# NetLogo-Mobile/Phy-Engine

Hardware: AMD Instinct MI355X
Metric: transient steps/sec (+ Newton iters/sec), 10k-node RC mesh (higher is better)
Workload: dtype f64

## Files before the change

### include/pe_hip.h

```cpp
#ifndef PE_HIP_H
#define PE_HIP_H

#include <stddef.h>
#include <stdint.h>

#ifdef __cplusplus
extern "C" {
#endif

typedef struct pe_hip_engine pe_hip_engine;

enum pe_hip_status
{
    PE_HIP_OK = 0,
    PE_HIP_ERR_ARG = -1,
    PE_HIP_ERR_NO_DEVICE = -2,
    PE_HIP_ERR_SINGULAR = -3,
    PE_HIP_ERR_NO_CONVERGENCE = -4,
    PE_HIP_ERR_INTERNAL = -5,
    PE_HIP_ERR_INACCURATE = -6
};

enum pe_hip_kind
{
// ... 59 lines not shown
} pe_hip_timings;

typedef struct pe_hip_info
{
    int rows, n_nodes, n_branches, batch;
    int nnz_a;
    long long nnz_lu;
    long long nnz_lu_stored;
    int n_fronts, max_front, tree_depth, n_row_swaps;
    double factor_flops;
    long long bytes_per_instance;
    int n_r, n_c, n_l, n_v, n_i, n_d;
    int nonlinear;
    int n_parts;
    int n_top_levels;
    int n_wavefronts;
    int lds_bytes;
    long long nnz_lu_stored_top;
    int n_wave_fronts;
    int n_quad_fronts;
    long long nnz_lu_stored_quad;
    int mid_top_limit, ew_grid, quad_lds_pad;
} pe_hip_info;

typedef struct pe_hip_run_stats
{
    long long steps;
    long long newton_iters;
    double gpu_ms;
    int n_launches;
    int n_failed;
    double dominant_ms;
    int dominant_launches;
} pe_hip_run_stats;

int pe_hip_device_count(void);
int pe_hip_create(int device, pe_hip_engine** out);
void pe_hip_destroy(pe_hip_engine* h);
const char* pe_hip_last_error(pe_hip_engine* h);

int pe_hip_solve_csr_real(pe_hip_engine* h, int n, int nnz, const int* row_ptr, const int* col_ind, const double* values,
                          const double* b, double* x, int copy_pattern, pe_hip_timings* out);

int pe_hip_solve_csr_complex(pe_hip_engine* h, int n, int nnz, const int* row_ptr, const int* col_ind, const double* values_re_im,
                             const double* b_re_im, double* x_re_im, int copy_pattern, pe_hip_timings* out);

const char* pe_hip_build_id(void);

int pe_hip_load_circuit(pe_hip_engine* h, int n_nodes, int n_branches, int batch, int n_tables, const pe_hip_device_table* tables);
int pe_hip_set_options(pe_hip_engine* h, const pe_hip_options* opt);
int pe_hip_get_info(pe_hip_engine* h, pe_hip_info* out);
int pe_hip_get_front_table(pe_hip_engine* h, int which, int capacity, int* pivots, int* updates, int* parent, int* kind, int* quad, int* mode,
                           int* n_children, int* n_own, int* n_fronts);

int pe_hip_set_knob(pe_hip_engine* h, const char* name, int value);
int pe_hip_get_knob(pe_hip_engine* h, const char* name, int* value, int* is_set);

int pe_hip_set_digital_drives(pe_hip_engine* h, int count, const int* node, const double* volt);

#define PE_HIP_OVERLAY_STEP 0
#define PE_HIP_OVERLAY_ITERATE 1
#define PE_HIP_OVERLAY_CONVERGED 2
#define PE_HIP_OVERLAY_VETO 100
#define PE_HIP_OVERLAY_AC 3
#define PE_HIP_OVERLAY_INSTANCE 4
typedef int (*pe_hip_overlay_fn)(void* user, int event, int mode, double t, double dt, const double* x, double* a_values, double* b_values);
int pe_hip_set_overlay(pe_hip_engine* h, int n_cells, const int* rows, const int* cols, const double* representative, int n_rhs, const int* rhs_rows,
                       int nonlinear, pe_hip_overlay_fn fn, void* user);

int pe_hip_update_param(pe_hip_engine* h, int kind, int index, int column, const double* values, int batched);

int pe_hip_set_time(pe_hip_engine* h, double t, double last_step);
int pe_hip_reset(pe_hip_engine* h);

int pe_hip_analyze_dc(pe_hip_engine* h, int mode, pe_hip_run_stats* stats);
int pe_hip_analyze_tr(pe_hip_engine* h, double dt, int nsteps, pe_hip_run_stats* stats);

typedef struct pe_hip_tr_control {
    double dt_init;
    double dt_min, dt_max;
    double lte_reltol, lte_abstol_v, lte_abstol_i;
    double trtol;
    long long max_steps;
    int source_breakpoints;
    int n_breakpoints; const double* breakpoints;
} pe_hip_tr_control;
typedef struct pe_hip_tr_adaptive_stats {
    long long n_accepted, n_rejected_lte, n_rejected_newton, n_at_dt_min;
    long long newton_iters_rejected;
    int n_analyses;
    double dt_smallest, dt_largest, t_end;
    pe_hip_run_stats run;
} pe_hip_tr_adaptive_stats;
int pe_hip_analyze_tr_adaptive(pe_hip_engine* h, double t_stop, const pe_hip_tr_control* c, pe_hip_tr_adaptive_stats* stats);
int pe_hip_get_tr_step_log(pe_hip_engine* h, long long first, int capacity, double* dt, int* outcome, long long* n_total);

int pe_hip_checkpoint_size(pe_hip_engine* h, size_t* bytes);
int pe_hip_checkpoint_save(pe_hip_engine* h, void* buffer, size_t capacity);
int pe_hip_checkpoint_load(pe_hip_engine* h, const void* buffer, size_t size);

int pe_hip_analyze_ac(pe_hip_engine* h, double omega, pe_hip_run_stats* stats);
int pe_hip_get_solution_ac(pe_hip_engine* h, int first_instance, int count, double* re, double* im);

typedef struct pe_hip_ac_sweep_stats {
    int n_points;
    int n_passes;
// ... 131 lines not shown
```

### phy-engine_amd/csrc/pe_device.hpp

```cpp
#pragma once
#include <cstddef>
#include <cstdint>

#include "pe_symbolic.hpp"

namespace pe
{
    enum : int
    {
        DV_ONE = 0,
        DV_GMIN = 1,
        DV_FIXED = 2
    };
    enum : int
    {
        PE_PROF = 96
    };

    enum : int
    {
        DP_IS_EFF = 0,
        DP_ISR_EFF,
        DP_UTE,
        DP_UTER,
// ... 101 lines not shown
        long long const *f_lptr, *f_uptr, *f_sptr;
        int const *row_src, *col_src;
        int const* row_dst{};
        unsigned char const* row_dyn{};
        int const *wave_ptr, *wave_list, *coop_ptr, *coop_list, *top_ptr, *top_list;
        int n_parts, n_top_levels, n_waves;
        int top_cnt[64];
        int top_wide[64]{};
        int lds_top_doubles{};
        int lds_mid_doubles{};
        int mid_top_limit{512}, ew_grid{}, quad_lds_pad{};
        int top_run_any_class{};
        int const* f_need{};
        int* active;
        int* flags;
        int high_occupancy;
        int keep_l21;
        int wave_m, wave_p, max_m, max_p;
        int lds_slot;
        int lds_sslot;
        int lds_bstack_off{};
        int const *f_wstack{}, *f_wpar{};
        int lds_wave_stage{}, lds_coop_stage{};
        int lds_top_stage{};
        int lds_solve_top_doubles{};
        int lds_doubles;
        int lds_solve_doubles;
        int lds_sslot_b{}, lds_bstack_off_b{}, lds_wave_stage_b{}, lds_solve_b_doubles{};
        int quad{};
        int const *q_prog{}, *q_lists{};
        unsigned char const* q_lane{};
        int const* q_bprog{};
        int quad_back{};
        int const *q2_prog{}, *q2_lists{};
        unsigned char const* q2_lane{};
        int n_mid{};
        int const* f_quad{};
        int const* f_kind{};
        long long q_zero_off{};
        int q_lds_stride{};
        int const* q_list{};
        int n_quads{};
        int probe_armed{};
        double v_abstol, v_reltol, i_abstol, i_reltol;
        int max_newton;
        int const *csr_rp, *csr_ci, *slot_e;
        double* xsave;
        double* rres;
        double* eta_acc;
        double residual_tol;
    };
    static_assert(offsetof(DevView, v_abstol) == offsetof(DevView, probe_armed) + sizeof(int), "probe_armed must fill the padding before v_abstol");

    struct ProbedView : DevView
    {
        ProbeView pr{};
    };
}
```

### phy-engine_amd/csrc/pe_engine.cpp

```cpp
#include "pe_engine_internal.hpp"

using namespace pe_eng;

namespace pe_eng PE_ENG_HIDDEN
{
    thread_local std::string g_create_error;

    int fail(pe_hip_engine* h, int code, std::string msg)
    {
        h->err = std::move(msg);
        return code;
    }

    double r_open_of(pe_hip_engine const* h) { return h->opt.r_open > 0.0 ? h->opt.r_open : 1e12; }

    void apply_options(pe_hip_engine* h, pe::DevView& V)
    {
        auto const& o = h->opt;
        V.v_abstol = o.v_abstol > 0.0 ? o.v_abstol : 1e-6;
        V.v_reltol = o.v_reltol > 0.0 ? o.v_reltol : 1e-3;
        V.i_abstol = o.i_abstol > 0.0 ? o.i_abstol : 1e-12;
        V.i_reltol = o.i_reltol > 0.0 ? o.i_reltol : V.v_reltol;
        V.max_newton = o.max_newton > 0 ? o.max_newton : 64;
        V.keep_l21 = (o.refactor_every_solve || V.nonlinear) ? 0 : 1;
// ... 376 lines not shown
        h->loaded = false;
    h->overlay = std::move(next);
    h->overlay_fn = fn;
    h->overlay_user = user;
    return PE_HIP_OK;
}

int pe_hip_set_digital_drives(pe_hip_engine* h, int count, const int* node, const double* volt)
{
    if(!h || count < 0 || (count > 0 && (!node || !volt))) return PE_HIP_ERR_ARG;
    ++h->param_epoch;
    if(h->loaded)
    {
        bool same = count == h->hc.n_drives;
        for(int k = 0; k < count && same; ++k) same = (node[k] == 0 ? -1 : node[k] - 1) == h->hc.drv_node[k];
        if(same)
        {
            HIPCHK(h, hipSetDevice(h->device));
            for(int k = 0; k < count; ++k)
            {
                std::vector<double> col(h->hc.batch, volt[k]);
                HIPCHK(h, hipMemcpy2D(h->V.dv + h->hc.dv_drv + k, h->hc.dv_len * sizeof(double), col.data(), sizeof(double), sizeof(double),
                                      h->hc.batch, hipMemcpyHostToDevice));
                h->hc.drv_volt[k] = volt[k];
            }
        }
        else
            h->loaded = false;
    }
    h->drv_node.assign(node, node + count);
    h->drv_volt.assign(volt, volt + count);
    return PE_HIP_OK;
}

int pe_hip_load_circuit(pe_hip_engine* h, int n_nodes, int n_branches, int batch, int n_tables, const pe_hip_device_table* tables)
{
    if(!h || (n_tables > 0 && !tables)) return PE_HIP_ERR_ARG;
    HIPCHK(h, hipSetDevice(h->device));
    h->loaded = false;
    h->sym_class = -1;
    h->fact_valid = false;
    h->a_static.clear();
    pe::m2_graphs_clear(h->graphs);
    probe_drop(h);
    tr_adaptive_drop(h);
    h->circ_pool.release();
    h->stats_scratch = nullptr;
    h->stats_doubles = 0;
    h->active_dev.clear();
    h->singular_rematched = false;
    h->sym_dt = 0.0;
    h->careful = false;
    h->n_refined = h->n_rematched = 0;
    h->sym_pool.release();
    ac_sweep_drop(h);
    dc_sweep_drop(h);
    if(h->ac.eng)
    {
        if(h->ac.d_xacc) (void)hipFree(h->ac.d_xacc);
        if(h->ac.d_b0) (void)hipFree(h->ac.d_b0);
        if(h->ac.d_worst) (void)hipFree(h->ac.d_worst);
        pe_hip_destroy(h->ac.eng);
        h->ac = pe_hip_engine::Ac{};
    }
    if(!pe::build_circuit(n_nodes, n_branches, batch, n_tables, tables, static_cast<int>(h->drv_node.size()), h->drv_node.data(),
                          h->drv_volt.data(), h->hc, h->overlay.empty() ? nullptr : &h->overlay))
        return fail(h, PE_HIP_ERR_ARG, "load_circuit: " + h->hc.error);
    return finish_load(h);
}


int pe_hip_get_info(pe_hip_engine* h, pe_hip_info* out)
{
    if(!h || !out || !h->loaded) return PE_HIP_ERR_ARG;
    std::memset(out, 0, sizeof(*out));
    auto const& hc = h->hc;
    out->rows = hc.rows;
    out->n_nodes = hc.n_nodes;
    out->n_branches = hc.n_branches;
    out->batch = hc.batch;
    out->nnz_a = static_cast<int>(hc.ci.size());
    out->n_r = hc.nR(); out->n_c = hc.nC(); out->n_l = hc.nL(); out->n_v = hc.nVdc() + hc.nVac() + hc.n_drives; out->n_i = hc.nIdc(); out->n_d = hc.nD();
    out->nonlinear = hc.nonlinear;
    if(h->sym_class >= 0)
    {
        out->nnz_lu = h->sym.nnz_LU;
        out->nnz_lu_stored = h->sym.nnz_LU_stored;
        out->n_fronts = h->sym.nfronts;
        out->max_front = h->sym.max_m;
        out->tree_depth = h->sym.tree_depth;
        out->n_parts = h->V.n_parts;
        out->n_top_levels = h->V.n_top_levels;
        out->n_wavefronts = h->V.n_waves;
        out->lds_bytes = h->V.lds_doubles * 8;
        for(int s = 0; s < h->sym.nfronts; ++s)
        {
            long long const stored = 2LL * h->sym.f_p[s] * h->sym.f_u[s] + static_cast<long long>(h->sym.f_p[s]) * h->sym.f_p[s];
            if(h->sym.f_kind[s] == 0) ++out->n_wave_fronts;
            if(h->V.quad && !h->sym.f_quad.empty() && h->sym.f_quad[s])
            {
                ++out->n_quad_fronts;
                out->nnz_lu_stored_quad += stored;
            }
        }
        for(int s = 0; s < h->sym.nfronts; ++s)
            if(h->sym.f_kind[s] == 2) out->nnz_lu_stored_top += 2LL * h->sym.f_p[s] * h->sym.f_u[s] + static_cast<long long>(h->sym.f_p[s]) * h->sym.f_p[s];
        out->n_row_swaps = h->sym.n_row_swaps;
        out->factor_flops = h->sym.flops;
        out->mid_top_limit = h->V.mid_top_limit;
        out->ew_grid = h->V.ew_grid;
        out->quad_lds_pad = h->V.quad_lds_pad;
    }
    out->bytes_per_instance = static_cast<long long>((h->circ_pool.bytes + h->sym_pool.bytes) / std::max(1, hc.batch));
    return PE_HIP_OK;
}

int pe_hip_get_front_table(pe_hip_engine* h, int which, int capacity, int* pivots, int* updates, int* parent, int* kind, int* quad, int* mode,
                           int* n_children, int* n_own, int* n_fronts)
{
    if(!h || !n_fronts || capacity < 0) return PE_HIP_ERR_ARG;
    pe::Symbolic const* S = nullptr;
    pe::DevView const* V = nullptr;
    if(which == 0 && h->loaded && h->sym_class >= 0) S = &h->sym, V = &h->V;
    else if(which == 1 && h->csr.have) S = &h->csr.sym, V = &h->csr.V;
    else if(which == 2 && h->csrz.have) S = &h->csrz.sym, V = &h->csrz.V;
    if(!S) return fail(h, PE_HIP_ERR_ARG, "get_front_table: no such analysis");
    auto at = [](std::vector<int> const& v, int s) { return static_cast<size_t>(s) < v.size() ? v[static_cast<size_t>(s)] : 0; };
    *n_fronts = S->nfronts;
    for(int s = 0; s < S->nfronts && s < capacity; ++s)
    {
        if(pivots) pivots[s] = S->f_p[s];
        if(updates) updates[s] = S->f_u[s];
        if(parent) parent[s] = S->f_parent[s];
        if(kind) kind[s] = at(S->f_kind, s);
        if(quad) quad[s] = (V->quad && at(S->f_quad, s)) ? 1 : 0;
        if(mode) mode[s] = at(S->f_mode, s);
        if(n_children) n_children[s] = S->f_child_ptr[s + 1] - S->f_child_ptr[s];
        if(n_own) n_own[s] = S->f_asm_ptr[s + 1] - S->f_asm_ptr[s];
    }
    return PE_HIP_OK;
}

int pe_hip_set_time(pe_hip_engine* h, double t, double last_step)
{
    if(!h || !h->loaded) return PE_HIP_ERR_ARG;
    HIPCHK(h, hipSetDevice(h->device));
    probe_disarm(h);
    std::vector<double> a(h->hc.batch, t), b(h->hc.batch, last_step);
    HIPCHK(h, hipMemcpy(h->V.t_now, a.data(), a.size() * sizeof(double), hipMemcpyHostToDevice));
    HIPCHK(h, hipMemcpy(h->V.last_step, b.data(), b.size() * sizeof(double), hipMemcpyHostToDevice));
    return PE_HIP_OK;
}

int pe_hip_reset(pe_hip_engine* h)
{
    if(!h || !h->loaded) return PE_HIP_ERR_ARG;
    HIPCHK(h, hipSetDevice(h->device));
    probe_disarm(h);
    ac_sweep_invalidate(h);
    auto const& hc = h->hc;
    size_t const B = static_cast<size_t>(hc.batch);
    auto& V = h->V;
    HIPCHK(h, hipMemset(V.x, 0, B * hc.rows * sizeof(double)));
    HIPCHK(h, hipMemset(V.c_hist, 0, std::max<size_t>(1, B * hc.nC()) * sizeof(double)));
    HIPCHK(h, hipMemset(V.c_prevg, 0, std::max<size_t>(1, B * hc.nC()) * sizeof(double)));
    HIPCHK(h, hipMemset(V.d_udlast, 0, std::max<size_t>(1, B * hc.nD()) * sizeof(double)));
    HIPCHK(h, hipMemset(V.d_geq, 0, std::max<size_t>(1, B * hc.nD()) * sizeof(double)));
    HIPCHK(h, hipMemset(V.d_hist, 0, std::max<size_t>(1, B * hc.nD()) * sizeof(double)));
    HIPCHK(h, hipMemset(V.d_prevg, 0, std::max<size_t>(1, B * hc.nD()) * sizeof(double)));
    HIPCHK(h, hipMemset(V.rl_engaged, 0, std::max<size_t>(1, B * hc.nRl()) * sizeof(int)));
    HIPCHK(h, hipMemset(V.t_now, 0, B * sizeof(double)));
    HIPCHK(h, hipMemset(V.last_step, 0, B * sizeof(double)));
    HIPCHK(h, hipMemset(V.status, 0, B * sizeof(int)));
    HIPCHK(h, hipMemset(V.n_steps, 0, B * sizeof(long long)));
    HIPCHK(h, hipMemset(V.n_iters, 0, B * sizeof(long long)));
    HIPCHK(h, hipMemset(V.trace_len, 0, sizeof(int)));
    HIPCHK(h, hipMemset(V.prof, 0, B * pe::PE_PROF * sizeof(long long)));
    h->fact_valid = false;
    h->a_static.clear();
    return PE_HIP_OK;
}

int pe_hip_get_solution(pe_hip_engine* h, int first, int count, double* x)
{
    if(!h || !h->loaded || !x || first < 0 || count < 0 || first + count > h->hc.batch) return PE_HIP_ERR_ARG;
    HIPCHK(h, hipSetDevice(h->device));
    HIPCHK(h, hipMemcpy(x, h->V.x + static_cast<size_t>(first) * h->hc.rows, static_cast<size_t>(count) * h->hc.rows * sizeof(double),
                        hipMemcpyDeviceToHost));
    return PE_HIP_OK;
}

int pe_hip_set_solution(pe_hip_engine* h, int first, int count, const double* x)
// ... 508 lines not shown
```

### phy-engine_amd/csrc/pe_engine_internal.hpp

```cpp
#pragma once
#define PE_ENG_HIDDEN __attribute__((visibility("hidden")))
#include <hip/hip_runtime_api.h>

#include <algorithm>
#include <chrono>
#include <cmath>
#include <cstdio>
#include <cstdlib>
#include <cstring>
#include <memory>
#include <string>
#include <vector>

#include "../../include/pe_hip.h"
#include "pe_ac.hpp"
#include "pe_ac_sweep.hpp"
#include "pe_circuit.hpp"
#include "pe_dc_sweep.hpp"
#include "pe_device.hpp"
#include "pe_kernels.hpp"
#include "pe_lte.hpp"
#include "pe_noise.hpp"
#include "pe_symbolic.hpp"

// ... 73 lines not shown
    bool careful{};
    long long n_refined{}, n_rematched{};
    int* pin_active{};
    int* pin_flags{};
    size_t pin_cap{};
    void* pub_host{};
    void* pub_dev{};
    size_t pub_cap{};
    unsigned long long pub_seq{};
    std::vector<int> active_dev;
    pe::M2GraphCache* graphs{};
    bool graph_mode{};
    double* stats_scratch{};
    size_t stats_doubles{};
    double* stats_pinned{};
    size_t stats_pinned_bytes{};
    struct Probes
    {
        Pool pool;
        bool configured{}, armed{};
        int n_probes{}, n_meas{}, capacity{}, stride{}, batch{};
        std::vector<int> kind;
        pe::ProbeView pv{};
        int* pin_accept{};
        size_t pin_cap{};
    } probe;
    struct TrAdaptive
    {
        Pool pool;
        bool allocated{};
        pe::StateCopy save{}, restore{};
        long long* shadow_iters{};
        double* hist{};
        unsigned long long* q_each{};
        pe::LteResult* result{};
        int n_pts{};
        int head{};
        double t_pts[3]{};
        std::vector<double> log_dt;
        std::vector<int> log_outcome;
    } tra;
    long long n_symbolic{};
    Pool circ_pool;
    Pool sym_pool;
    pe::Symbolic sym;
    int sym_class{-1};
    double sym_dt{};
    pe::DevView V{};
    bool fact_valid{};
    double fact_dt{};
    std::vector<char> a_static;
    double a_static_dt{-1.0};
    double analyze_ms{};

    struct Ac
    {
        pe_hip_engine* eng{};
        pe::AcCircuit circ;
        bool built{};
        double sym_omega{-1.0};
        std::vector<int> b_ptr0, b_src0;
        int rhs0{};
        std::vector<double> x;
        double *d_xacc{}, *d_b0{}, *d_worst{};
        size_t d_len{};
        struct Sweep
        {
            pe_hip_engine* eng{};
            int P{};
            Pool pass_pool;
            Pool circ_pool;
            Pool res_pool;
            size_t res_len{};
            bool rows_on_device{};
            int* d_keep{};
            size_t keep_cap{};
            pe::AcSweepView V{};
            long long bytes_per_instance{};
            std::vector<int> rows;
            bool valid{};
            int n_points{}, n_keep{}, batch{};
            std::vector<double> res;
        } sweep;
    } ac;
    struct Noise
    {
        Ac sys;
        bool have_pair{};
        int out_pos{-1}, out_neg{-1};
        bool table_built{}, table_on_device{};
        std::vector<pe::NoiseSource> src;
        std::vector<int> kind, index, part;
        Pool src_pool;
        Pool pass_pool;
        size_t partial_len{};
        Pool res_pool;
        size_t res_len{};
        double* d_res{};
        pe::NoiseView V{};
        bool valid{};
        bool kept{};
        bool have_density{};
        int n_points{}, batch{};
        std::vector<double> res;
        std::vector<double> integrated;
    } noise;
// ... 35 lines not shown
        bool have{};
        bool on_these_values{};
        std::vector<int> rp2, ci2, pos;
        std::vector<double> vals, rhs, x;
        double *d_xacc{}, *d_b0{}, *d_worst{};
    } csrz;
};

static inline int hip_error_code(hipError_t e)
{
    return (e == hipErrorNoDevice || e == hipErrorInvalidDevice || e == hipErrorInsufficientDriver) ? PE_HIP_ERR_NO_DEVICE : PE_HIP_ERR_INTERNAL;
}

#define HIPCHK(h, expr)                                                                             \
    do {                                                                                            \
        hipError_t e__ = (expr);                                                                    \
        if(e__ != hipSuccess)                                                                       \
        {                                                                                           \
            (h)->err = std::string("HIP error: ") + hipGetErrorString(e__) + " at " #expr;          \
            return hip_error_code(e__);                                                             \
        }                                                                                           \
    } while(0)

static inline char const* csr_pattern_error(int n, int nnz, int const* row_ptr, int const* col_ind)
{
    if(n > 0 && (row_ptr[0] != 0 || row_ptr[n] != nnz)) return "row_ptr[0] != 0 or row_ptr[n] != nnz";
    for(int i = 0; i < n; ++i)
    {
        if(row_ptr[i + 1] < row_ptr[i]) return "row_ptr is not monotone";
        for(int e = row_ptr[i]; e < row_ptr[i + 1]; ++e)
            if(col_ind[e] < 0 || col_ind[e] >= n || (e > row_ptr[i] && col_ind[e] <= col_ind[e - 1])) return "column indices out of range or not sorted inside a row";
    }
    return nullptr;
}

namespace pe_eng PE_ENG_HIDDEN
{
    extern thread_local std::string g_create_error;

    int fail(pe_hip_engine* h, int code, std::string msg);
    double r_open_of(pe_hip_engine const* h);
    void apply_options(pe_hip_engine* h, pe::DevView& V);
    int stats_chunks(int batch);
    int finish_load(pe_hip_engine* h);
    void fill_static_dv(pe_hip_engine const* h, std::vector<double>& dv);
    int collect_stats(pe_hip_engine* h, std::vector<long long> const& steps0, std::vector<long long> const& iters0, pe_hip_run_stats* st);
    int snapshot_counters(pe_hip_engine* h, std::vector<long long>& s0, std::vector<long long>& i0);
    bool split_launch(pe_hip_engine const* h);
    int env_int0(char const* name, int def);
    int knob(pe_hip_engine const* h, char const* name, int def);
    int upload_symbolic(pe_hip_engine* h, Pool& pool, pe::Symbolic& S, pe::SymbolicOptions const& so, pe::DevView& V, int batch);
    pe::SymbolicOptions symbolic_options(pe_hip_engine const* h, int batch_in, int rows, int panel_reserve = 384, int force_resident = 0);
    int analyze_fitting(pe_hip_engine* h, int batch, int geometry_rows, int n, int const* rp, int const* ci, double const* vals, pe::Symbolic& S,
                        pe::SymbolicOptions& so);
    int ensure_symbolic(pe_hip_engine* h, bool tr, double dt);
    pe::ProbedView probe_view(pe_hip_engine const* h);
    void probe_disarm(pe_hip_engine* h);
    void probe_drop(pe_hip_engine* h);
    int probe_record_step(pe_hip_engine* h, std::vector<int> const& accepted, double t);
    struct CkPart
    {
        void* ptr;
        size_t bytes;
    };
    std::vector<CkPart> ck_parts(pe_hip_engine* h);
    void tr_adaptive_drop(pe_hip_engine* h);
    void ac_sweep_drop(pe_hip_engine* h);
    inline void ac_sweep_invalidate(pe_hip_engine* h)
    {
        h->ac.sweep.valid = false;
        h->noise.valid = false;
    }
    long long sweep_memory_budget();
    constexpr long long SWEEP_MAX_INSTANCES = 65535;
    void dc_sweep_drop(pe_hip_engine* h);
    int dc_solve(pe_hip_engine* h, int mode, pe_hip_run_stats* st, bool clear_status);
    bool has_overlay(pe_hip_engine const* h);
    int overlay_call(pe_hip_engine* h, int event, int mode, double t, double dt, int b = 0);
    int overlay_call_all(pe_hip_engine* h, int event, int mode, double t, double dt, std::vector<int> const* mask);
}
```

### phy-engine_amd/csrc/pe_engine_newton.cpp

```cpp
#include "pe_engine_internal.hpp"

using namespace pe_eng;

namespace pe_eng PE_ENG_HIDDEN
{
    int overlay_call(pe_hip_engine* h, int event, int mode, double t, double dt, int b)
    {
        auto const& hc = h->hc;
        h->ov_x.resize(static_cast<size_t>(hc.rows));
        HIPCHK(h, hipStreamSynchronize(h->stream));
        if(hc.batch > 1 && h->overlay_fn(h->overlay_user, PE_HIP_OVERLAY_INSTANCE, b, t, dt, nullptr, nullptr, nullptr) != 0)
            return fail(h, PE_HIP_ERR_INTERNAL, "host-stamp overlay: the callback refused PE_HIP_OVERLAY_INSTANCE (it does not support batches)");
        if(hc.rows) HIPCHK(h, hipMemcpy(h->ov_x.data(), h->V.x + static_cast<size_t>(b) * hc.rows, static_cast<size_t>(hc.rows) * sizeof(double), hipMemcpyDeviceToHost));
        bool const iter = event == PE_HIP_OVERLAY_ITERATE;
        h->ov_a.assign(static_cast<size_t>(hc.n_ov_a), 0.0);
        h->ov_b.assign(static_cast<size_t>(hc.n_ov_b), 0.0);
        int const orc = h->overlay_fn(h->overlay_user, event, mode, t, dt, h->ov_x.data(), iter ? h->ov_a.data() : nullptr, iter ? h->ov_b.data() : nullptr);
        if(event == PE_HIP_OVERLAY_CONVERGED && orc == PE_HIP_OVERLAY_VETO) return PE_HIP_OVERLAY_VETO;
        if(orc != 0) return fail(h, PE_HIP_ERR_INTERNAL, "host-stamp overlay: a model hook failed");
        if(iter)
        {
            double* dv = h->V.dv + static_cast<size_t>(b) * h->V.dv_len;
            if(hc.n_ov_a) HIPCHK(h, hipMemcpy(dv + hc.dv_ova, h->ov_a.data(), static_cast<size_t>(hc.n_ov_a) * sizeof(double), hipMemcpyHostToDevice));
            if(hc.n_ov_b) HIPCHK(h, hipMemcpy(dv + hc.dv_ovb, h->ov_b.data(), static_cast<size_t>(hc.n_ov_b) * sizeof(double), hipMemcpyHostToDevice));
// ... 165 lines not shown
    }
    int publish_and_wait(pe_hip_engine* h, std::vector<int>& flags, std::vector<double>* eta)
    {
        size_t const B = flags.size();
        if(int const rc = ensure_published(h, B); rc != PE_HIP_OK) return rc;
        auto const dev = pub_view(h->pub_dev, B);
        unsigned long long const seq = ++h->pub_seq;
        HIPCHK(h, pe::launch_m2_publish(h->stream, h->V, dev.flags, dev.eta, dev.seq, seq));
        return wait_published(h, flags, eta, seq);
    }

    int m2_check_residuals(pe_hip_engine* h, M2State& S, std::vector<int>& result, int& n_active, std::vector<double> const& published,
                           std::vector<char>& owes)
    {
        int const B = h->hc.batch;
        std::vector<double> eta(static_cast<size_t>(B) * 4);
        bool first = published.size() == eta.size();
        auto pull_eta = [&]() -> int
        {
            if(first)
            {
                eta = published;
                first = false;
                return PE_HIP_OK;
            }
            HIPCHK(h, hipMemcpy(eta.data(), h->V.eta_acc, eta.size() * sizeof(double), hipMemcpyDeviceToHost));
            return PE_HIP_OK;
        };
        auto bad = [&](int b)
        {
            double const* n = &eta[4 * static_cast<size_t>(b)];
            double const den = n[1] * n[2] + n[3];
            double const e = den > 0.0 ? n[0] / den : (n[0] > 0.0 ? INFINITY : 0.0);
            return !(e <= h->V.residual_tol);
        };
        auto checked = [&](int b) { return S.active[b] && !(S.flags[b] & 5) && !(h->hc.nonlinear && (S.flags[b] & 2)); };
        auto owed = [&](int b) { return S.active[b] && !(S.flags[b] & 5) && h->hc.nonlinear && (S.flags[b] & 2) && owes[static_cast<size_t>(b)]; };
        bool any = false;
        for(int b = 0; b < B && !any; ++b) any = checked(b) || owed(b);
        if(!any) return PE_HIP_OK;
        if(int const rc = pull_eta(); rc != PE_HIP_OK) return rc;
        std::vector<int> todo;
        for(int b = 0; b < B; ++b)
            if((checked(b) && bad(b)) || owed(b)) todo.push_back(b);
        if(todo.empty()) return PE_HIP_OK;
        for(int b: todo) owes[static_cast<size_t>(b)] = 1;
        std::vector<int> mask(B);
        for(int round = 0; round < 2 && !todo.empty(); ++round)
        {
            std::fill(mask.begin(), mask.end(), 0);
            for(int b: todo) mask[b] = 1;
            if(int const urc = upload_active(h, mask); urc != PE_HIP_OK) return urc;
            HIPCHK(h, pe::launch_m2_refine(h->stream, h->V));
            HIPCHK(h, hipStreamSynchronize(h->stream));
            if(int const rc = pull_eta(); rc != PE_HIP_OK) return rc;
            std::vector<int> fl(B);
            HIPCHK(h, hipMemcpy(fl.data(), h->V.flags, B * sizeof(int), hipMemcpyDeviceToHost));
            std::vector<int> still;
            for(int b: todo)
            {
                S.flags[b] = fl[b];
                if((fl[b] & 5) == 0 && bad(b)) still.push_back(b);
                else
                    ++h->n_refined;
            }
            todo.swap(still);
        }
        for(int b: todo)
        {
            result[b] = PE_HIP_ERR_INACCURATE;
            S.active[b] = 0;
            --n_active;
        }
        return PE_HIP_OK;
    }

    int m2_point(pe_hip_engine* h, M2State& S, int mode, double t, double last_step, bool do_factor, std::vector<int>& result, int& launches,
                 double const* companion_dt = nullptr, bool a_static_ok = false)
    {
        int const B = h->hc.batch;
        result.assign(B, 0);
        int n_active = 0;
        for(int b = 0; b < B; ++b)
        {
            S.active[b] = S.status[b] == PE_HIP_OK ? 1 : 0;
            n_active += S.active[b];
        }
        int const max_it = h->hc.nonlinear ? h->V.max_newton : 1;
        std::vector<char> owes_refinement(static_cast<size_t>(B), 0);
        static bool const use_publish = env_int0("PHY_ENGINE_HIP_PUBLISH", 1) != 0;
        bool const graph_mode = use_publish && knob(h, "GRAPH", B <= 32 ? 1 : 0) != 0;
        if(graph_mode != h->graph_mode)
        {
            h->graph_mode = graph_mode;
            h->active_dev.clear();
        }
        if(graph_mode && !h->graphs) h->graphs = pe::m2_graphs_create();
        for(int it = 0; it < max_it && n_active > 0; ++it)
        {
            if(has_overlay(h))
                if(int const rc = overlay_call_all(h, PE_HIP_OVERLAY_ITERATE, mode, t, last_step, &S.active); rc != PE_HIP_OK) return rc;
            if(int const urc = upload_active(h, S.active); urc != PE_HIP_OK) return urc;
            static bool const full_stamp = env_int0("PHY_ENGINE_HIP_FULL_STAMP", 0) != 0;
            int const dyn = full_stamp ? 0 : (it > 0 ? 1 : (a_static_ok ? 2 : 0));
            bool const comp = it == 0 && companion_dt != nullptr;
            std::vector<double> eta_now;
            if(graph_mode)
            {
                if(int const prc = ensure_published(h, static_cast<size_t>(B)); prc != PE_HIP_OK) return prc;
                auto const dev = pub_view(h->pub_dev, static_cast<size_t>(B));
                unsigned long long const seq = ++h->pub_seq;
                HIPCHK(h, pe::launch_m2_iteration_graph(h->stream, h->graphs, h->V, mode, t, last_step, do_factor, dyn, comp, companion_dt ? *companion_dt : 0.0, dev.flags,
                                                        dev.eta, dev.seq, seq));
                ++launches;
                if(int const prc = wait_published(h, S.flags, &eta_now, seq); prc != PE_HIP_OK) return prc;
            }
            else
            {
                HIPCHK(h, pe::launch_m2_iteration(h->stream, h->V, mode, t, last_step, do_factor, h->evk0, h->evk1, dyn, comp,
                                                  companion_dt ? *companion_dt : 0.0));
                ++launches;
                if(use_publish)
                {
                    if(int const prc = publish_and_wait(h, S.flags, &eta_now); prc != PE_HIP_OK) return prc;
                }
                else if(int const drc = download_flags(h, S.flags); drc != PE_HIP_OK)
                    return drc;
                float kms = 0.f;
                if(hipEventElapsedTime(&kms, h->evk0, h->evk1) == hipSuccess)
                {
                    h->dominant_ms += kms;
                    ++h->dominant_launches;
                }
            }
            if(h->V.residual_tol > 0.0)
                if(int const rrc = m2_check_residuals(h, S, result, n_active, eta_now, owes_refinement); rrc != PE_HIP_OK) return rrc;
            for(int b = 0; b < B; ++b)
            {
                if(!S.active[b]) continue;
                int const f = S.flags[b];
                if(f & 8) return fail(h, PE_HIP_ERR_INTERNAL, "a front's LDS layout exceeds the LDS of the launch that ran it (launch plan / layout mismatch)");
                if(f & 5) result[b] = PE_HIP_ERR_SINGULAR;
                else if(!h->hc.nonlinear || !(f & 2))
                {
                    if(has_overlay(h) && h->hc.nonlinear)
                    {
                        int const crc = overlay_call(h, PE_HIP_OVERLAY_CONVERGED, mode, t, last_step, b);
                        if(crc == PE_HIP_OVERLAY_VETO) continue;
                        if(crc != PE_HIP_OK) return crc;
                    }
                    result[b] = it + 1;
                }
                else
                    continue;
                S.active[b] = 0;
                --n_active;
            }
        }
        for(int b = 0; b < B; ++b)
            if(S.active[b])
            {
                result[b] = PE_HIP_ERR_NO_CONVERGENCE;
                S.active[b] = 0;
            }
        return PE_HIP_OK;
    }

    int run_m2_tr(pe_hip_engine* h, double dt, int nsteps, int& launches, std::vector<int> const* only = nullptr, bool retry = true)
    {
        M2State S;
        int rc = m2_pull(h, S);
        if(rc != PE_HIP_OK) return rc;
        int const B = h->hc.batch;
// ... 128 lines not shown
                failed.push_back(b);
                any_inaccurate = any_inaccurate || status[b] == PE_HIP_ERR_INACCURATE;
            }
        if(failed.empty() || attempt >= 2) return PE_HIP_OK;
        if(!any_inaccurate) h->singular_rematched = true;
        if(any_inaccurate && attempt == 0 && (!h->careful || !split_launch(h))) h->careful = true;
        else
        {
            int const b = failed[0];
            size_t const nnz = h->hc.ci.size();
            std::vector<double> tmp(nnz);
            HIPCHK(h, hipMemcpy(tmp.data(), h->V.aval + static_cast<size_t>(b) * nnz, nnz * sizeof(double), hipMemcpyDeviceToHost));
            h->sym_values_override.assign(nnz, 0.0);
            for(size_t e = 0; e < nnz; ++e)
            {
                double const v = std::fabs(tmp[e]);
                h->sym_values_override[h->sym.asm_slot[e]] = v <= 1.7976931348623157e308 ? v : 1.0;
            }
            h->sym_class = -1;
            int const rc = ensure_symbolic(h, tr, dt);
            h->sym_values_override.clear();
            if(rc != PE_HIP_OK) return rc;
            ++h->n_rematched;
        }
        for(int b: failed) status[b] = PE_HIP_OK;
        HIPCHK(h, hipMemcpy(h->V.status, status.data(), B * sizeof(int), hipMemcpyHostToDevice));
        for(int b: failed)
        {
            int const owe = tr ? nsteps - static_cast<int>(s1[b] - steps0[b]) : 1;
            auto it = std::find_if(groups.begin(), groups.end(), [&](auto const& g) { return g.first == owe; });
            if(it == groups.end())
            {
                groups.emplace_back(owe, std::vector<int>(B, 0));
                it = groups.end() - 1;
            }
            it->second[b] = 1;
        }
        return PE_HIP_OK;
    }
}

#if !defined(__HIPCC__)
    #include "pe_probe.hpp"
namespace pe
{
    namespace
    {
        struct ProbeHostTeam
        {
            int tid() const { return 0; }
            int size() const { return 1; }
            void sync() const {}
        };
    }
    hipError_t launch_probe_arm(hipStream_t, ProbedView const& V)
    {
        for(int b = 0; b < V.batch; ++b) probe_arm(ProbeHostTeam{}, V, b);
        return hipSuccess;
    }
    hipError_t launch_probe_record(hipStream_t, ProbedView const& V, double t)
    {
        for(int b = 0; b < V.batch; ++b)
            if(V.pr.accept[b]) probe_record(ProbeHostTeam{}, V, b, t);
        return hipSuccess;
    }
    hipError_t launch_tr_lte(hipStream_t, DevView const& V, LteView const& L)
    {
        *L.result = LteResult{};
        for(int b = 0; b < V.batch; ++b)
        {
            int nonfinite = 0;
            unsigned long long const u = lte_partial(ProbeHostTeam{}, V, L, b, nonfinite);
            if(L.test)
            {
                L.q_each[b] = u;
                if(u > L.result->q) L.result->q = u;
            }
            L.result->n_nonfinite += nonfinite;
            if(V.status[b] != 0) ++L.result->n_failed;
            L.result->iters_spent += L.iters_now[b] - L.iters_before[b];
        }
        return hipSuccess;
    }
    hipError_t launch_tr_history_push(hipStream_t, DevView const& V, double* hist, int slot)
    {
        lte_history_push(ProbeHostTeam{}, V, hist, slot);
        return hipSuccess;
    }
    hipError_t launch_tr_state_copy(hipStream_t, StateCopy const& S)
    {
        for(int p = 0; p < S.n; ++p)
            if(S.bytes[p]) std::memcpy(S.dst[p], S.src[p], S.bytes[p]);
        return hipSuccess;
    }
    hipError_t launch_dc_sweep_fill(hipStream_t, DevView const& V, DcSweepView const& S)
    {
        dc_sweep_fill(ProbeHostTeam{}, V, S);
        return hipSuccess;
    }
    hipError_t launch_dc_sweep_seed(hipStream_t, DevView const& V, DcSweepView const& S, bool from_main)
    {
        for(int q = 0; q < V.batch; ++q) dc_sweep_seed(ProbeHostTeam{}, V, S, q, from_main);
        return hipSuccess;
    }
    hipError_t launch_dc_sweep_classify(hipStream_t, DevView const& V, DcSweepView const& S, bool reseed)
    {
// ... 844 lines not shown
```

### phy-engine_amd/csrc/pe_engine_policy.cpp

```cpp
#include "pe_engine_internal.hpp"
#include "pe_top_plan.hpp"

using namespace pe_eng;

namespace pe_eng PE_ENG_HIDDEN
{
    bool split_launch(pe_hip_engine const* h)
    {
        int const v = knob(h, "SPLIT", -1);
        if(v == 1) return true;
        if(v == 0) return false;
        if(h->overlay_fn && (h->hc.n_ov_a || h->hc.n_ov_b)) return true;
        if(h->careful) return true;
        return h->V.n_parts > 1 || h->hc.rows >= 3000;
    }

    int geometry_batch(pe_hip_engine const* h, int batch)
    {
        int const v = knob(h, "GEOMETRY_BATCH", 0);
        return v > 0 ? v : batch;
    }


    long long panel_need(int p, int u) { return static_cast<long long>(pe::pe_ld(p + u)) * p + static_cast<long long>(pe::pe_ld(p)) * u; }
// ... 245 lines not shown
        if(so.wave_slot > 0 && so.n_waves * so.wave_slot > lds_doubles) so.wave_slot = 0;
        if(so.wave_slot == 0)
            while(static_cast<long long>(so.n_waves) * so.wave_m * (pe::pe_ld(so.wave_m) + 1) > lds_doubles && so.wave_m > 8) --so.wave_m;
        so.wave_p = std::min(so.wave_p, so.wave_m);
        so.absorb_m = std::min(so.absorb_m, so.wave_m);
        so.panel_doubles = std::max<long long>(lds_doubles - panel_reserve, lds_doubles / 2);
        so.panel_reserve = lds_doubles - so.panel_doubles;
        return so;
    }

    void regroup_wide_top(pe_hip_engine* h, int batch, int geometry_rows, int n, int const* rp, int const* ci, double const* vals, pe::Symbolic& S,
                          pe::SymbolicOptions& so)
    {
        so.big_unknowns = nullptr;
        bool const split = geometry_rows >= 3000 && knob(h, "SPLIT", -1) != 0 && S.n_parts > 1;
        if(!split || knob(h, "TOP_BIG", 1) == 0 || knob(h, "WIDE_TOP", 1) == 0 || knob(h, "TOP_CHAIN_LDS", 1) == 0) return;
        int const gb = geometry_batch(h, batch), levels = static_cast<int>(S.top_ptr.size()) - 1;
        std::vector<char> big(static_cast<size_t>(n), 0);
        int marked = 0;
        bool const half_knob = knob(h, "TOP_BIG", 1) != 2;
        long long const half_wgs = std::max(0, knob(h, "TOP_HALF_WGS", 2048));
        for(int l = 0; l < levels; ++l)
        {
            long long const wgs = static_cast<long long>(S.top_ptr[l + 1] - S.top_ptr[l]) * gb;
            int const cls = (!so.shared_cu || wgs <= std::max(0, knob(h, "TOP_WIDE_WGS", 320))) ? 1 : ((half_knob && wgs <= half_wgs) ? 2 : 0);
            if(cls == 0) continue;
            for(int k = S.top_ptr[l]; k < S.top_ptr[l + 1]; ++k)
            {
                int const s = S.top_list[k];
                for(int c = S.f_col0[s]; c < S.f_col0[s] + S.f_p[s]; ++c) big[static_cast<size_t>(S.col_src[c])] = static_cast<char>(cls);
                ++marked;
            }
        }
        if(marked < 2) return;
        pe::SymbolicOptions so2 = so;
        so2.big_unknowns = &big;
        so2.max_pivots_top = std::clamp(knob(h, "TOP_MAX_PIVOTS", 64), 1, 64);
        long long const whole_cu = h->lds_limit / 8 - 160 - 8;
        long long const behind = std::max<long long>(so.panel_reserve, S.max_m + 8 + 512);
        so2.panel_doubles_top = whole_cu - 2 - behind;
        so2.panel_doubles_mid = so.shared_cu ? (h->lds_limit / 8 - 160) / 2 - 8 - 2 - behind : 0;
        pe::Symbolic S2;
        if(!pe::analyze(n, rp, ci, vals, so2, S2)) return;
        if(static_cast<int>(S2.top_ptr.size()) - 1 > 64 || S2.max_m + 8 > so.panel_reserve || S2.n_parts != S.n_parts) return;
        for(int s = 0; s < S2.nfronts; ++s)
            if(lds_class(S2, so2, s) != 0 && S2.f_kind[s] != 2) return;
        S = std::move(S2);
        so.max_pivots_top = so2.max_pivots_top;
        so.panel_doubles_top = so2.panel_doubles_top;
        so.panel_doubles_mid = so2.panel_doubles_mid;
    }

    int analyze_fitting(pe_hip_engine* h, int batch, int geometry_rows, int n, int const* rp, int const* ci, double const* vals, pe::Symbolic& S,
                        pe::SymbolicOptions& so)
    {
        so = symbolic_options(h, batch, geometry_rows);
        for(int attempt = 0;; ++attempt)
        {
            if(!pe::analyze(n, rp, ci, vals, so, S))
                return fail(h, S.structurally_singular ? PE_HIP_ERR_SINGULAR : PE_HIP_ERR_INTERNAL, "symbolic analysis: " + S.error);
            bool const too_deep = static_cast<int>(S.top_ptr.size()) - 1 > 64;
            bool const fits = S.max_m + 8 <= so.panel_reserve;
            if(fits && !too_deep)
            {
                regroup_wide_top(h, batch, geometry_rows, n, rp, ci, vals, S, so);
                return PE_HIP_OK;
            }
            if(attempt == 2) return fail(h, PE_HIP_ERR_INTERNAL, "symbolic analysis: a front of order " + std::to_string(S.max_m) + " does not fit the LDS of a CU");
            so = symbolic_options(h, batch, geometry_rows, std::max(384, S.max_m + 72), attempt == 1 ? 1 : 0);
            if(too_deep) so.n_parts = 1;
        }
    }

    int ensure_symbolic(pe_hip_engine* h, bool tr, double dt)
    {
        int const cls = tr ? 1 : 0;
        bool const dt_moved = tr && h->sym_dt > 0.0 && dt > 0.0 && (dt > 10.0 * h->sym_dt || dt < 0.1 * h->sym_dt) && h->sym_values_override.empty();
        if(h->sym_class == cls && !dt_moved) return PE_HIP_OK;
        if(tr) h->sym_dt = dt;
        auto const t0 = clk::now();
        std::vector<double> av;
        if(!h->sym_values_override.empty()) av = h->sym_values_override;
        else
        {
            pe::estimate_values(h->hc, tr, dt, h->opt.g_min, r_open_of(h), av);
            if(char const* k = std::getenv("PHY_ENGINE_HIP_TEST_BLIND_MATCH"); k && *k == '1') std::fill(av.begin(), av.end(), 1.0);
        }
        pe::SymbolicOptions so{};
        {
            int const rc = analyze_fitting(h, h->hc.batch, h->hc.rows, h->hc.rows, h->hc.rp.data(), h->hc.ci.data(), av.data(), h->sym, so);
            if(rc != PE_HIP_OK)
            {
                h->sym_class = -1;
                return rc;
            }
        }
        if(char const* dump = std::getenv("PHY_ENGINE_HIP_DUMP_SCHEDULE"); dump && *dump == '1')
        {
            auto const& S = h->sym;
            int nk[4]{};
            for(int s = 0; s < S.nfronts; ++s) ++nk[S.f_kind[s]];
            std::fprintf(stderr, "[pe_hip] schedule: %d fronts (%d wave, %d cooperative, %d top, %d mid), %d parts, %d top levels\n", S.nfronts, nk[0], nk[1],
                         nk[2], nk[3], S.n_parts, static_cast<int>(S.top_ptr.size()) - 1);
            if(S.quad)
                std::fprintf(stderr, "[pe_hip]   lane-group kernel: LDS stack %d doubles per instance holds %lld of %lld update-matrix doubles of the wave fronts\n",
                             S.q_lds_doubles, S.q_lds_kept, S.q_lds_total);
            if(S.quad)
            {
                std::fprintf(stderr, "[pe_hip]   wave-front lists (fronts):");
                for(size_t L = 0; 2 * L + 1 < S.q_lists.size(); ++L) std::fprintf(stderr, " %d", S.q_lists[2 * L + 1]);
                std::fprintf(stderr, "\n[pe_hip]   MID lists (fronts):");
                for(size_t L = 0; 2 * L + 1 < S.q2_lists.size(); ++L) std::fprintf(stderr, " %d", S.q2_lists[2 * L + 1]);
                std::fprintf(stderr, "\n");
                for(int s = 0; s < S.nfronts; ++s)
                    if(S.f_kind[s] == 3 && dump[1] == '4')
                        std::fprintf(stderr, "[pe_hip]   mid front %d: %dx%d children %d parent %d(kind %d)\n", s, S.f_p[s] + S.f_u[s], S.f_p[s], S.f_child_ptr[s + 1] - S.f_child_ptr[s],
                                     S.f_parent[s], S.f_parent[s] >= 0 ? S.f_kind[S.f_parent[s]] : -1);
            }
            for(int kind = 0; kind < 2; ++kind)
            {
                long long cnt[3]{}, su2[3]{}, spanel[3]{};
                long long const cap = kind == 0 ? std::max<long long>(S.wave_panel_doubles, 1) : so.panel_doubles;
                for(int s = 0; s < S.nfronts; ++s)
                {
                    if(S.f_kind[s] != kind) continue;
                    long long const p = S.f_p[s], u = S.f_u[s], m = p + u;
                    int const nch = S.f_child_ptr[s + 1] - S.f_child_ptr[s];
                    int const mode = m * m <= cap ? 0 : (nch == 1 && S.f_u[S.f_child[S.f_child_ptr[s]]] == m ? 2 : 1);
                    ++cnt[mode];
                    su2[mode] += u * u;
                    spanel[mode] += m * p + p * u;
                }
                std::fprintf(stderr, "[pe_hip]   %s fronts (cap ~%lld doubles): whole %lld (S %lld, panels %lld) | panel+pull %lld (S %lld, panels %lld) | chain link %lld (S %lld, panels %lld)\n",
                             kind == 0 ? "wave" : "cooperative", cap, cnt[0], su2[0], spanel[0], cnt[1], su2[1], spanel[1], cnt[2], su2[2], spanel[2]);
            }
            if(dump[1] == '3')
                for(int s = 0; s < S.nfronts; ++s)
                    if(S.f_kind[s] == 0) std::fprintf(stderr, "[pe_hip]   wave front %d: %dx%d children %d\n", s, S.f_p[s] + S.f_u[s], S.f_p[s], S.f_child_ptr[s + 1] - S.f_child_ptr[s]);
            if(dump[1] == '2')
                for(int s = 0; s < S.nfronts; ++s)
                    if(S.f_kind[s] == 1) std::fprintf(stderr, "[pe_hip]   coop front %d: %dx%d children %d\n", s, S.f_p[s] + S.f_u[s], S.f_p[s], S.f_child_ptr[s + 1] - S.f_child_ptr[s]);
            for(std::size_t l = 0; l + 1 < S.top_ptr.size(); ++l)
            {
                std::fprintf(stderr, "[pe_hip]   top level %zu:", l);
                for(int k = S.top_ptr[l]; k < S.top_ptr[l + 1]; ++k) std::fprintf(stderr, " %dx%d", S.f_p[S.top_list[k]] + S.f_u[S.top_list[k]], S.f_p[S.top_list[k]]);
                std::fprintf(stderr, "\n");
            }
        }
        pe::m2_graphs_clear(h->graphs);
        h->sym_pool.release();
        int const rc = upload_symbolic(h, h->sym_pool, h->sym, so, h->V, h->hc.batch);
        if(rc != PE_HIP_OK) return rc;
        h->active_dev.clear();
        if(char const* dump = std::getenv("PHY_ENGINE_HIP_DUMP_SCHEDULE"); dump && *dump == '1')
        {
            auto const& S = h->sym;
            std::fprintf(stderr, "[pe_hip]   top fronts, LDS layout (0 whole, 1 panels, 2 chain link, 3 chain link continued in LDS; * = 16-wavefront level, %d doubles):", h->V.lds_top_doubles);
            for(std::size_t l = 0; l + 1 < S.top_ptr.size(); ++l)
                for(int k = S.top_ptr[l]; k < S.top_ptr[l + 1]; ++k) std::fprintf(stderr, " %d%s", S.f_mode[S.top_list[k]], h->V.top_wide[l] ? "*" : "");
            std::fprintf(stderr, "\n");
        }
        if(char const* dump = std::getenv("PHY_ENGINE_HIP_DUMP_SCHEDULE"); dump && *dump == '1')
        {
            auto const& S = h->sym;
            long long hist[8]{}, tiles = 0;
            for(int s = 0; s < S.nfronts; ++s)
            {
                if(S.f_kind[s] == 0 || S.f_mode[s] != 1) continue;
                int const u = S.f_u[s], nt = (u + 15) / 16, ch0 = S.f_child_ptr[s], ch1 = S.f_child_ptr[s + 1];
                for(int tj = 0; tj < nt; ++tj)
                    for(int ti = 0; ti < nt; ++ti)
                    {
                        int n = 0;
                        for(int c = ch0; c < ch1; ++c)
                        {
                            unsigned const mk = S.f_bmask[static_cast<size_t>(c)];
                            n += static_cast<int>(((mk >> std::min(ti, 31)) & (mk >> std::min(tj, 31))) & 1u);
                        }
                        ++hist[std::min(n, 7)];
                        ++tiles;
                    }
            }
            std::fprintf(stderr, "[pe_hip]   panel-layout Schur tiles by children pulled (0..7+) of %lld:", tiles);
            for(long long v: hist) std::fprintf(stderr, " %lld", v);
            std::fprintf(stderr, "\n");
        }
        if(char const* dump = std::getenv("PHY_ENGINE_HIP_DUMP_SCHEDULE"); dump && *dump == '1')
            std::fprintf(stderr, "[pe_hip]   LDS plan (doubles): factor %d, solves %d, backward %d (wave slot %d = t %d + stage %d + 64 + stack %d), wave front slot %d\n", h->V.lds_doubles,
                         h->V.lds_solve_doubles, h->V.lds_solve_b_doubles, h->V.lds_sslot, h->V.wave_m, h->V.lds_wave_stage, h->V.lds_sslot - h->V.lds_bstack_off, h->V.lds_slot);
        {
            auto const& S = h->sym;
            auto const& hc = h->hc;
            size_t const nnz = hc.ci.size();
            std::vector<int> ptr2(nnz + 1, 0), src2;
            src2.reserve(hc.a_src.size());
            for(size_t e = 0; e < nnz; ++e)
            {
                int const slot = S.asm_slot[e];
                src2.insert(src2.end(), hc.a_src.begin() + hc.a_ptr[slot], hc.a_src.begin() + hc.a_ptr[slot + 1]);
                ptr2[e + 1] = static_cast<int>(src2.size());
            }
            if(src2.empty()) src2.push_back(0);
            HIPCHK(h, h->sym_pool.upload(h->V.a_ptr, ptr2));
            HIPCHK(h, h->sym_pool.upload(h->V.a_src, src2));
            h->V.dyn_a = h->V.dyn_b = nullptr;
            h->V.n_dyn_a = h->V.n_dyn_b = 0;
            if(hc.nonlinear)
            {
                std::vector<char> const dyn = pe::dynamic_dv_mask(hc);
                std::vector<int> da, db;
                for(size_t e = 0; e < nnz; ++e)
                    for(int k = ptr2[e]; k < ptr2[e + 1]; ++k)
                        if(dyn[static_cast<size_t>(src2[k] >> 1)])
                        {
                            da.push_back(static_cast<int>(e));
                            break;
                        }
                for(int r = 0; r < hc.rows; ++r)
                    for(int k = hc.b_ptr[r]; k < hc.b_ptr[r + 1]; ++k)
                        if(dyn[static_cast<size_t>(hc.b_src[k] >> 1)])
                        {
                            db.push_back(r);
                            break;
                        }
                h->V.n_dyn_a = static_cast<int>(da.size());
                h->V.n_dyn_b = static_cast<int>(db.size());
                if(da.empty()) da.push_back(0);
                if(db.empty()) db.push_back(0);
                HIPCHK(h, h->sym_pool.upload(h->V.dyn_a, da));
                HIPCHK(h, h->sym_pool.upload(h->V.dyn_b, db));
                std::vector<unsigned char> rd(static_cast<size_t>(std::max(1, hc.rows)), 0);
                for(int k = 0; k < h->V.n_dyn_b; ++k) rd[static_cast<size_t>(db[static_cast<size_t>(k)])] = 1;
                HIPCHK(h, h->sym_pool.upload(h->V.row_dyn, rd));
            }
            h->V.asm_slot = nullptr;
            std::vector<int> slot_e(nnz, 0);
            for(size_t e = 0; e < nnz; ++e) slot_e[S.asm_slot[e]] = static_cast<int>(e);
            HIPCHK(h, h->sym_pool.upload(h->V.slot_e, slot_e));
        }
        h->sym_class = cls;
        h->fact_valid = false;
        h->a_static.clear();
        h->analyze_ms = ms_since(t0);
        ++h->n_symbolic;
        return PE_HIP_OK;
    }

}
```

### phy-engine_amd/csrc/pe_front.hpp

```cpp
#pragma once
#include "pe_device.hpp"

#include <cassert>
#include <cmath>

#if defined(__HIPCC__)
    #define PE_DEV __device__ __forceinline__
#else
    #define PE_DEV inline
#endif
#if defined(PE_ASM_MARKS) && defined(__HIPCC__)
    #define PE_MARK(name) asm volatile("; PE_MARK " name ::: "memory")
#else
    #define PE_MARK(name) ((void)0)
#endif
#include "pe_probe.hpp"

namespace pe
{
    enum : int
    {
        MODE_OP = 0,
        MODE_DC = 1,
        MODE_TR = 4,
// ... 347 lines not shown
    {
        for(int base = lo + t0; base < n; base += UN * T)
        {
            int slot[UN];
            int e[UN], end[UN];
            double acc[UN];
#pragma unroll
            for(int q = 0; q < UN; ++q)
            {
                int const k = base + q * T;
                bool const ok = k < n;
                int const s = ok ? (list ? list[k] : k) : 0;
                slot[q] = s;
                e[q] = ok ? ptr[s] : 0;
                end[q] = ok ? ptr[s + 1] : 0;
                acc[q] = 0.0;
            }
            bool more = true;
            while(more)
            {
                more = false;
                int sr[UN];
#pragma unroll
                for(int q = 0; q < UN; ++q) sr[q] = e[q] < end[q] ? src[e[q]] : -1;
                double v[UN];
#pragma unroll
                for(int q = 0; q < UN; ++q) v[q] = dv[sr[q] >= 0 ? sr[q] >> 1 : 0];
#pragma unroll
                for(int q = 0; q < UN; ++q)
                    if(sr[q] >= 0)
                    {
                        acc[q] = (sr[q] & 1) ? acc[q] - v[q] : acc[q] + v[q];
                        ++e[q];
                        more = more || e[q] < end[q];
                    }
            }
#pragma unroll
            for(int q = 0; q < UN; ++q)
                if(base + q * T < n)
                {
                    out[slot[q]] = acc[q];
                    if(out2) out2[perm[slot[q]]] = acc[q];
                }
        }
    }

    template <class Team>
    PE_DEV void stamp(Team const& tm, DevView const& V, int b)
    {
        double const* dv = V.dv + static_cast<long long>(b) * V.dv_len;
        gather_contributions(tm.tid(), tm.size(), V.a_ptr, V.a_src, dv, V.aval + static_cast<long long>(b) * V.nnzA, 0, V.nnzA);
        gather_contributions(tm.tid(), tm.size(), V.b_ptr, V.b_src, dv, V.rhs + static_cast<long long>(b) * V.rows, 0, V.rows);
    }
    PE_DEV void stamp_dynamic_chunk(DevView const& V, int b, int g, int G, int t0, int T, bool with_w = false, bool rhs_full = false)
    {
        double const* dv = V.dv + static_cast<long long>(b) * V.dv_len;
        double* w = with_w ? V.w + static_cast<long long>(b) * V.rows : nullptr;
        auto range = [&](int n, int& lo, int& hi)
        {
            int const c = (n + G - 1) / G;
            lo = g * c < n ? g * c : n;
            hi = lo + c < n ? lo + c : n;
        };
        int lo, hi;
        range(V.n_dyn_a, lo, hi);
        gather_contributions<PE_STAMP_UN>(t0, T, V.a_ptr, V.a_src, dv, V.aval + static_cast<long long>(b) * V.nnzA, lo, hi, V.dyn_a);
        if(rhs_full)
        {
            range(V.rows, lo, hi);
            gather_contributions<PE_STAMP_UN>(t0, T, V.b_ptr, V.b_src, dv, V.rhs + static_cast<long long>(b) * V.rows, lo, hi, nullptr, w, V.row_dst);
            return;
        }
        range(V.n_dyn_b, lo, hi);
        gather_contributions<PE_STAMP_UN>(t0, T, V.b_ptr, V.b_src, dv, V.rhs + static_cast<long long>(b) * V.rows, lo, hi, V.dyn_b, w, V.row_dst);
        if(with_w)
        {
            double const* rhs = V.rhs + static_cast<long long>(b) * V.rows;
            range(V.rows, lo, hi);
            for(int k = lo + t0; k < hi; k += T)
            {
                int const r = V.row_src[k];
                if(!V.row_dyn[r]) w[k] = rhs[r];
            }
        }
    }
    PE_DEV void stamp_chunk(DevView const& V, int b, int g, int G, int t0, int T, bool with_w = false)
    {
        double const* dv = V.dv + static_cast<long long>(b) * V.dv_len;
        double* w = with_w ? V.w + static_cast<long long>(b) * V.rows : nullptr;
        auto range = [&](int n, int& lo, int& hi)
        {
            int const c = (n + G - 1) / G;
            lo = g * c < n ? g * c : n;
            hi = lo + c < n ? lo + c : n;
        };
        int lo, hi;
        range(V.nnzA, lo, hi);
        gather_contributions<PE_STAMP_UN>(t0, T, V.a_ptr, V.a_src, dv, V.aval + static_cast<long long>(b) * V.nnzA, lo, hi);
        range(V.rows, lo, hi);
        gather_contributions<PE_STAMP_UN>(t0, T, V.b_ptr, V.b_src, dv, V.rhs + static_cast<long long>(b) * V.rows, lo, hi, nullptr, w, V.row_dst);
    }


    PE_DEV bool bad_pivot(double piv) { return piv == 0.0 || !(fabs(piv) <= 1.7976931348623157e308); }

    PE_DEV int fdiv(int idx, float rcp) { return static_cast<int>((static_cast<float>(idx) + 0.5f) * rcp); }

    template <int UN>
    PE_DEV void stage_copy(double* dst, double const* src, int n, int t0, int T)
    {
        for(int base = t0; base < n; base += UN * T)
        {
            double r[UN];
#pragma unroll
            for(int q = 0; q < UN; ++q)
            {
                int const idx = base + q * T;
                r[q] = idx < n ? src[idx] : 0.0;
            }
#pragma unroll
            for(int q = 0; q < UN; ++q)
            {
                int const idx = base + q * T;
                if(idx < n) dst[idx] = r[q];
            }
        }
    }

    struct ChainState
    {
        double* img{};
        int ld{};
        double* g{};
    };

// ... 757 lines not shown
                    if(q < nq && j < u) acc += ug[q] * t[p + j];
                }
            }
            else
                for(int q = 0; q < (nq < UQ ? nq : UQ); ++q)
                {
                    int const j = jg + G * q;
                    if(j < u) acc += Ug[i + static_cast<long long>(j) * p] * t[p + j];
                }
            for(int q = UQ; q < nq; ++q)
            {
                int const j = jg + G * q;
                if(j < u) acc += Ug[i + static_cast<long long>(j) * p] * t[p + j];
            }
            part[jg * R + i] = acc;
        }
        tm.sync_lds();
        for(int i = t0; i < p; i += T)
        {
            double acc = i == t0 ? wi : w[c0 + i];
            for(int g2 = 0; g2 < G; ++g2) acc -= part[g2 * R + i];
            t[i] = acc;
        }
        tm.sync_lds();
        tm.for_each_wave(
            [&](int wv, int lane, int)
            {
                if(wv == 0) tm.tri_upper(t, Ub, p, p, 0, lane);
            });
        tm.sync_lds();
        for(int i = t0; i < p; i += T) w[c0 + i] = t[i];
    }

    template <class Team>
    PE_DEV void forward_part(Team const& tm, DevView const& V, int b, int part, double* lds)
    {
        int const* wp = V.wave_ptr + part * (V.n_waves + 1);
        tm.for_each_wave(
            [&](int wv, int lane, int NL)
            {
                auto wt = tm.wave_team(lane);
                double* sc = lds + static_cast<long long>(wv) * V.lds_sslot;
                int const q1 = tm.uniform(wp[wv + 1]);
                for(int q = tm.uniform(wp[wv]); q < q1; ++q) front_forward(wt, V, b, V.wave_list[q], sc, V.wave_m, V.lds_wave_stage);
            });
        tm.sync();
        for(int q = V.coop_ptr[part]; q < V.coop_ptr[part + 1]; ++q) front_forward(tm, V, b, V.coop_list[q], lds, V.max_m, V.lds_coop_stage);
    }

    template <class Team>
    PE_DEV void backward_part(Team const& tm, DevView const& V, int b, int part, double* lds)
    {
        int const* wp = V.wave_ptr + part * (V.n_waves + 1);
        long long const cbw0 = tm.clock();
        for(int q = V.coop_ptr[part + 1] - 1; q >= V.coop_ptr[part]; --q) front_backward(tm, V, b, V.coop_list[q], lds, V.max_m, V.lds_coop_stage);
        tm.sync();
        if(V.prof && tm.tid() == 0 && part == 0) V.prof[b * PE_PROF + 3] += tm.clock() - cbw0;
        tm.for_each_wave(
            [&](int wv, int lane, int NL)
            {
                auto wt = tm.wave_team(lane);
                double* sc = lds + static_cast<long long>(wv) * V.lds_sslot_b;
                int const q0 = tm.uniform(wp[wv]);
                for(int q = tm.uniform(wp[wv + 1]) - 1; q >= q0; --q)
                {
                    int const sq = tm.uniform(V.wave_list[q]);
                    if(V.quad_back && V.f_quad[sq]) continue;
                    int const pq = V.f_p[sq], mq = pq + V.f_u[sq];
                    if(pq <= 64 && mq <= V.wave_m && pq * pq <= V.lds_wave_stage_b) front_backward_lean(wt, V, b, sq, sc);
                    else
                    {
                        front_backward(wt, V, b, sq, sc, V.wave_m, V.lds_wave_stage_b);
                        double const* wb = V.w + static_cast<long long>(b) * V.rows;
                        double* tq = sc + V.lds_bstack_off_b + V.f_wstack[sq];
                        int const* rows = V.f_rows + V.f_rows_ptr[sq];
                        for(int i = wt.tid(); i < mq; i += wt.size()) tq[i] = i < pq ? wb[V.f_col0[sq] + i] : wb[rows[i - pq]];
                        wt.sync_lds();
                    }
                }
            });
        tm.sync();
    }

    template <class Team>
    PE_DEV void permute_rhs(Team const& tm, DevView const& V, int b)
    {
        double const* rhs = V.rhs + static_cast<long long>(b) * V.rows;
        double* w = V.w + static_cast<long long>(b) * V.rows;
        for(int k = tm.tid(); k < V.rows; k += tm.size()) w[k] = rhs[V.row_src[k]];
        tm.sync();
    }

    template <class Team>
    PE_DEV void solve_all(Team const& tm, DevView const& V, int b, double* lds, bool forward_done)
    {
        int const T = tm.size(), t0 = tm.tid();
        double* w = V.w + static_cast<long long>(b) * V.rows;
        double* x = V.x + static_cast<long long>(b) * V.rows;
        if(!forward_done) permute_rhs(tm, V, b);
        long long const c0 = tm.clock();
        if(!forward_done) forward_part(tm, V, b, 0, lds);
        backward_part(tm, V, b, 0, lds);
        if(V.prof && t0 == 0)
        {
            V.prof[b * PE_PROF + 5] += tm.clock() - c0;
        }
// ... 193 lines not shown
```

### phy-engine_amd/csrc/pe_kernels.hip

```cpp
#include <hip/hip_runtime.h>

#include <cstdlib>
#include <cstring>
#include <mutex>
#include <type_traits>
#include <unordered_map>
#include <vector>

#include "pe_front.hpp"
#include "pe_ac_sweep.hpp"
#include "pe_dc_sweep.hpp"
#include "pe_noise.hpp"
#include "pe_lte.hpp"
#include "pe_kernels.hpp"
#include "pe_quad.hpp"
#include "pe_top_plan.hpp"

namespace pe
{
    struct WaveOps
    {
        __device__ __forceinline__ void wave_fence() const
        {
            __builtin_amdgcn_fence(__ATOMIC_RELEASE, "workgroup");
// ... 489 lines not shown
    {
        int const b = static_cast<int>(blockIdx.x);
        if(b >= V.batch) return;
        HipTeam tm;
        int st = ST_OK;
        if(do_factor)
        {
            permute_rhs(tm, V, b);
            if(!factor_all(tm, V, b, pe_lds, true)) st = ST_SINGULAR;
        }
        if(st == ST_OK)
        {
            solve_all(tm, V, b, pe_lds, do_factor != 0);
            double const* x = V.x + static_cast<long long>(b) * V.rows;
            int nonfinite = 0;
            for(int r = tm.tid(); r < V.rows; r += tm.size())
                if(!(fabs(x[r]) <= 1.7976931348623157e308)) nonfinite = 1;
            if(tm.sync_or(nonfinite)) st = ST_SINGULAR;
        }
        if(tm.tid() == 0) V.status[b] = st;
    }

    struct GridTeam
    {
        __device__ __forceinline__ int tid() const { return static_cast<int>(blockIdx.x * blockDim.x + threadIdx.x); }
        __device__ __forceinline__ int size() const { return static_cast<int>(gridDim.x * blockDim.x); }
    };

    __global__ void __launch_bounds__(256) k_m2_companion(DevView V, double dt)
    {
        int const b = static_cast<int>(blockIdx.y);
        if(!V.active[b]) return;
        companion_update(GridTeam{}, V, b, dt);
    }

    __global__ void __launch_bounds__(256) k_m2_eval(DevView V, int mode, double t, double last_step, int dynamic_only, int companion_dt_set, double companion_dt)
    {
        int const b = static_cast<int>(blockIdx.y);
        if(!V.active[b]) return;
        GridTeam tm;
        if(companion_dt_set) companion_update(tm, V, b, companion_dt);
        double const* x = V.x + static_cast<long long>(b) * V.rows;
        double* xp = V.xprev + static_cast<long long>(b) * V.rows;
        for(int r = tm.tid(); r < V.rows; r += tm.size()) xp[r] = x[r];
        eval_devices(tm, V, b, mode, t, last_step, dynamic_only != 0);
        if(tm.tid() == 0)
        {
            V.flags[b] = 0;
            if(V.eta_acc)
                for(int k = 0; k < 4; ++k) V.eta_acc[4 * b + k] = 0.0;
        }
    }

    __global__ void __launch_bounds__(256) k_m2_stamp(DevView V, int dynamic_only)
    {
        int const b = static_cast<int>(blockIdx.y);
        if(!V.active[b]) return;
        if(dynamic_only) stamp_dynamic_chunk(V, b, static_cast<int>(blockIdx.x), static_cast<int>(gridDim.x), static_cast<int>(threadIdx.x), static_cast<int>(blockDim.x), true, dynamic_only == 2);
        else
            stamp_chunk(V, b, static_cast<int>(blockIdx.x), static_cast<int>(gridDim.x), static_cast<int>(threadIdx.x), static_cast<int>(blockDim.x), true);
    }

    __device__ __forceinline__ bool lds_overrun(DevView const& V, int b, int s, int lds_doubles)
    {
        if(V.f_need[s] <= lds_doubles - 2) return false;
        if(threadIdx.x == 0) atomicOr(V.flags + b, 8);
        return true;
    }

    template <int MINW>
    __global__ void __launch_bounds__(PE_THREADS, MINW) k_m2_factor_parts(DevView V)
    {
        int const b = static_cast<int>(blockIdx.x);
        if(!V.active[b]) return;
        HipTeam tm;
        long long const t_start = V.prof ? tm.clock() : 0;
        if(!factor_part(tm, V, b, static_cast<int>(blockIdx.y), pe_lds, true) && tm.tid() == 0) atomicOr(V.flags + b, 4);
        if(V.prof && tm.tid() == 0 && blockIdx.y < 4)
        {
            long long* q = V.prof + b * PE_PROF + 48 + 3 * static_cast<int>(blockIdx.y);
            q[0] = t_start;
            q[1] = tm.clock();
            q[2] = (static_cast<long long>(__builtin_amdgcn_s_getreg(6164)) << 32) | static_cast<unsigned>(__builtin_amdgcn_s_getreg(63492));
        }
    }

    template <int MINW>
    __global__ void __launch_bounds__(PE_THREADS, MINW) k_m2_factor_top(DevView V, int level, int nlev, int lds_doubles)
    {
        int const b = static_cast<int>(blockIdx.y);
        if(!V.active[b]) return;
        HipTeam tm;
        for(int l = level; l < level + nlev; ++l)
        {
            int const s = V.top_list[V.top_ptr[l] + static_cast<int>(blockIdx.x)];
            if(lds_overrun(V, b, s, lds_doubles)) return;
            if(!front_factor(tm, V, b, s, pe_lds, lds_doubles - 2, 0, true))
            {
                if(tm.tid() == 0) atomicOr(V.flags + b, 4);
                return;
            }
        }
    }

    __global__ void __launch_bounds__(1024) k_m2_factor_top_wide(DevView V, int level, int nlev, int lds_doubles)
    {
        int const b = static_cast<int>(blockIdx.y);
        if(!V.active[b]) return;
        HipTeam tm;
        ChainState cs;
        for(int l = level; l < level + nlev; ++l)
        {
            int const s = V.top_list[V.top_ptr[l] + static_cast<int>(blockIdx.x)];
            if(lds_overrun(V, b, s, lds_doubles)) return;
            if(!front_factor<HipTeam, true>(tm, V, b, s, pe_lds, lds_doubles - 2, 0, true, &cs))
            {
                if(tm.tid() == 0) atomicOr(V.flags + b, 4);
                return;
            }
        }
    }

    __global__ void __launch_bounds__(512, 4) k_m2_factor_top_mid(DevView V, int level, int nlev, int lds_doubles)
    {
        int const b = static_cast<int>(blockIdx.y);
        if(!V.active[b]) return;
        HipTeam tm;
        for(int l = level; l < level + nlev; ++l)
        {
            int const s = V.top_list[V.top_ptr[l] + static_cast<int>(blockIdx.x)];
            if(lds_overrun(V, b, s, lds_doubles)) return;
            if(!front_factor(tm, V, b, s, pe_lds, lds_doubles - 2, 0, true))
            {
                if(tm.tid() == 0) atomicOr(V.flags + b, 4);
                return;
            }
        }
    }

    __global__ void __launch_bounds__(256) k_m2_winit(DevView V)
    {
        int const b = static_cast<int>(blockIdx.y);
        if(!V.active[b]) return;
        GridTeam tm;
        double const* rhs = V.rhs + static_cast<long long>(b) * V.rows;
        double* w = V.w + static_cast<long long>(b) * V.rows;
        for(int k = tm.tid(); k < V.rows; k += tm.size()) w[k] = rhs[V.row_src[k]];
    }

    template <int MINW>
    __global__ void __launch_bounds__(PE_THREADS, MINW) k_m2_solve_parts(DevView V, int backward)
    {
        int const b = static_cast<int>(blockIdx.x);
        if(!V.active[b]) return;
        HipTeam tm;
        if(backward) backward_part(tm, V, b, static_cast<int>(blockIdx.y), pe_lds);
        else
            forward_part(tm, V, b, static_cast<int>(blockIdx.y), pe_lds);
    }

    __global__ void __launch_bounds__(256, 8) k_m2_backward_parts(DevView V)
    {
        int const b = static_cast<int>(blockIdx.x);
        if(!V.active[b]) return;
        HipTeam tm;
        backward_part(tm, V, b, static_cast<int>(blockIdx.y), pe_lds);
    }

    template <int MINW>
    __global__ void __launch_bounds__(PE_THREADS, MINW) k_m2_solve_top(DevView V, int level, int nlev, int backward)
    {
        int const b = static_cast<int>(blockIdx.y);
        if(!V.active[b]) return;
        HipTeam tm;
        for(int i = 0; i < nlev; ++i)
        {
            int const l = backward ? level + nlev - 1 - i : level + i;
            int const s = V.top_list[V.top_ptr[l] + static_cast<int>(blockIdx.x)];
            if(backward) front_backward(tm, V, b, s, pe_lds, V.max_m, V.lds_top_stage);
            else
                front_forward(tm, V, b, s, pe_lds, V.max_m, V.lds_top_stage);
        }
    }

    __global__ void __launch_bounds__(256) k_m2_finish(DevView V)
    {
        int const b = static_cast<int>(blockIdx.y);
        if(!V.active[b]) return;
        GridTeam tm;
        double const* w = V.w + static_cast<long long>(b) * V.rows;
        double* x = V.x + static_cast<long long>(b) * V.rows;
        double const* xp = V.xprev + static_cast<long long>(b) * V.rows;
        int bits = 0;
        for(int k = tm.tid(); k < V.rows; k += tm.size())
        {
            int const r = V.col_src[k];
            double const xn = w[k];
            x[r] = xn;
            if(!(fabs(xn) <= 1.7976931348623157e308)) bits |= 1;
            bool const node = r < V.n_nodes;
// ... 216 lines not shown
    static hipError_t set_lds(void const* fn, size_t bytes)
    {
        static std::mutex mu;
        static std::unordered_map<unsigned long long, size_t> allowed;
        int dev = 0;
        if(hipError_t const e = hipGetDevice(&dev); e != hipSuccess) return e;
        unsigned long long const key = (static_cast<unsigned long long>(reinterpret_cast<uintptr_t>(fn)) * 1000003ull) ^ static_cast<unsigned long long>(dev + 1);
        std::lock_guard<std::mutex> lock(mu);
        auto it = allowed.find(key);
        if(it != allowed.end() && bytes <= it->second) return hipSuccess;
        hipError_t const e = hipFuncSetAttribute(fn, hipFuncAttributeMaxDynamicSharedMemorySize, static_cast<int>(bytes));
        if(e == hipSuccess) allowed[key] = bytes;
        return e;
    }

    hipError_t launch_tr_steps(hipStream_t st, DevView const& V, double dt, int nsteps, bool reuse)
    {
        size_t const lds = static_cast<size_t>(V.lds_doubles) * sizeof(double);
        if(V.probe_armed)
        {
            auto const fn = V.high_occupancy ? &k_tr_steps<4, true> : &k_tr_steps<2, true>;
            hipError_t e = set_lds(reinterpret_cast<void const*>(fn), lds);
            if(e != hipSuccess) return e;
            hipLaunchKernelGGL(fn, dim3(V.batch), dim3(V.n_waves * 64), lds, st, static_cast<ProbedView const&>(V), dt, nsteps, reuse ? 1 : 0);
            return hipGetLastError();
        }
        auto const fn = V.high_occupancy ? &k_tr_steps<4, false> : &k_tr_steps<2, false>;
        hipError_t e = set_lds(reinterpret_cast<void const*>(fn), lds);
        if(e != hipSuccess) return e;
        hipLaunchKernelGGL(fn, dim3(V.batch), dim3(V.n_waves * 64), lds, st, V, dt, nsteps, reuse ? 1 : 0);
        return hipGetLastError();
    }

    hipError_t launch_dc_point(hipStream_t st, DevView const& V, int mode)
    {
        size_t const lds = static_cast<size_t>(V.lds_doubles) * sizeof(double);
        auto const fn = V.high_occupancy ? &k_dc_point<4> : &k_dc_point<2>;
        hipError_t e = set_lds(reinterpret_cast<void const*>(fn), lds);
        if(e != hipSuccess) return e;
        hipLaunchKernelGGL(fn, dim3(V.batch), dim3(V.n_waves * 64), lds, st, V, mode);
        return hipGetLastError();
    }

    static int grid_per_instance(DevView const& V)
    {
        if(V.ew_grid > 0) return V.ew_grid;
        int const by_rows = (V.rows + 2047) / 2048, fine = (V.rows + 255) / 256, want = 1280 / (V.batch > 0 ? V.batch : 1);
        int g = by_rows > (want < fine ? want : fine) ? by_rows : (want < fine ? want : fine);
        return g < 1 ? 1 : (g > 64 ? 64 : g);
    }

    template <int MINW>
    static hipError_t m2_sequence(hipStream_t st, DevView const& V, int mode, double t, double last_step, bool do_factor, hipEvent_t ev0, hipEvent_t ev1, bool refine,
                                  int stamp_mode = 0, bool companion = false, double companion_dt = 0.0)
    {
        bool const have_lists = V.dyn_a && V.dyn_b;
        int const eval_dyn = (stamp_mode == 1 && have_lists) ? 1 : 0, stamp_dyn = have_lists ? stamp_mode : 0;
        size_t const lds = static_cast<size_t>(V.lds_doubles) * sizeof(double);
        size_t const lds_s = static_cast<size_t>(V.lds_solve_doubles) * sizeof(double);
        size_t const lds_st = static_cast<size_t>(V.lds_solve_top_doubles) * sizeof(double);
        {
            hipError_t e = set_lds(reinterpret_cast<void const*>(&k_m2_factor_parts<MINW>), lds);
            if(e == hipSuccess) e = set_lds(reinterpret_cast<void const*>(&k_m2_factor_top<MINW>), lds);
            if(e == hipSuccess) e = set_lds(reinterpret_cast<void const*>(&k_m2_factor_top_wide), static_cast<size_t>(V.lds_top_doubles) * sizeof(double));
            if(e == hipSuccess) e = set_lds(reinterpret_cast<void const*>(&k_m2_factor_top_mid), std::max(lds, static_cast<size_t>(V.lds_mid_doubles) * sizeof(double)));
            if(e == hipSuccess) e = set_lds(reinterpret_cast<void const*>(&k_m2_solve_parts<MINW>), lds_s);
            if(e == hipSuccess) e = set_lds(reinterpret_cast<void const*>(&k_m2_solve_top<MINW>), lds_st);
            if(e != hipSuccess) return e;
        }
        int const B = V.batch, T = V.n_waves * 64;
        int const G = grid_per_instance(V);
        auto run = [&](int l) { return top_run(V, l); };
        auto run_down = [&](int l)
        {
            int n = 1;
            if(V.top_cnt[l] == 1)
                while(l - n >= 0 && V.top_cnt[l - n] == 1) ++n;
            return n;
        };
        if(!refine)
        {
            hipLaunchKernelGGL(k_m2_eval, dim3(G, B), dim3(256), 0, st, V, mode, t, last_step, eval_dyn, companion ? 1 : 0, companion_dt);
            hipLaunchKernelGGL(k_m2_stamp, dim3(G, B), dim3(256), 0, st, V, stamp_dyn);
        }
        else
            hipLaunchKernelGGL(k_m2_winit, dim3(G, B), dim3(256), 0, st, V);
        if(do_factor)
        {
            if(ev0) (void)hipEventRecord(ev0, st);
            if(V.quad && V.n_quads > 0)
            {
                size_t const qlds = std::max(static_cast<size_t>(std::max(0, V.quad_lds_pad)), static_cast<size_t>(V.q_lds_stride) * 32);
                if(qlds > 0)
                {
                    hipError_t const e = set_lds(reinterpret_cast<void const*>(&k_m2_factor_quads), qlds);
                    if(e != hipSuccess) return e;
                }
                hipLaunchKernelGGL(k_m2_factor_quads, dim3(V.n_quads * V.n_parts * V.n_waves), dim3(64), qlds, st, V);
                if(V.n_mid > 0) hipLaunchKernelGGL(k_m2_factor_mid, dim3(V.n_quads * V.n_parts * V.n_waves), dim3(64), 0, st, V);
            }
            hipLaunchKernelGGL(k_m2_factor_parts<MINW>, dim3(B, V.n_parts), dim3(T), lds, st, V);
            if(ev1) (void)hipEventRecord(ev1, st);
            for_each_top_launch(V, B, MINW == 4 && T == 256, V.mid_top_limit,
                                [&](TopLaunch const& t)
                                {
                                    dim3 const grid(V.top_cnt[t.level], B);
                                    size_t const bytes = static_cast<size_t>(t.lds_doubles) * sizeof(double);
                                    int const cap = static_cast<int>(t.lds_doubles);
                                    if(t.kind == 1) hipLaunchKernelGGL(k_m2_factor_top_wide, grid, dim3(1024), bytes, st, V, t.level, t.nlev, cap);
                                    else if(t.kind != 0)
                                        hipLaunchKernelGGL(k_m2_factor_top_mid, grid, dim3(512), bytes, st, V, t.level, t.nlev, cap);
                                    else
                                        hipLaunchKernelGGL(k_m2_factor_top<MINW>, grid, dim3(T), bytes, st, V, t.level, t.nlev, cap);
                                });
        }
        else
        {
            hipLaunchKernelGGL(k_m2_solve_parts<MINW>, dim3(B, V.n_parts), dim3(T), lds_s, st, V, 0);
            for(int l = 0; l < V.n_top_levels; l += run(l)) hipLaunchKernelGGL(k_m2_solve_top<MINW>, dim3(V.top_cnt[l], B), dim3(T), lds_st, st, V, l, run(l), 0);
        }
        for(int l = V.n_top_levels - 1; l >= 0;)
        {
            int const n = run_down(l);
            hipLaunchKernelGGL(k_m2_solve_top<MINW>, dim3(V.top_cnt[l], B), dim3(T), lds_st, st, V, l - n + 1, n, 1);
            l -= n;
        }
        if(!do_factor && ev0) (void)hipEventRecord(ev0, st);
        size_t const lds_b = static_cast<size_t>(V.lds_solve_b_doubles) * sizeof(double);
        if(T <= 256)
        {
            hipError_t const e = set_lds(reinterpret_cast<void const*>(&k_m2_backward_parts), lds_b);
            if(e != hipSuccess) return e;
            hipLaunchKernelGGL(k_m2_backward_parts, dim3(B, V.n_parts), dim3(T), lds_b, st, V);
        }
        else
            hipLaunchKernelGGL(k_m2_solve_parts<MINW>, dim3(B, V.n_parts), dim3(T), lds_b, st, V, 1);
        if(V.quad_back && V.n_quads > 0) hipLaunchKernelGGL(k_m2_backward_quads, dim3(V.n_quads * V.n_parts * V.n_waves), dim3(64), 0, st, V);
        if(!do_factor && ev1) (void)hipEventRecord(ev1, st);
        if(!refine)
        {
            hipLaunchKernelGGL(k_m2_finish, dim3(G, B), dim3(256), 0, st, V);
            if(V.residual_tol > 0.0) hipLaunchKernelGGL(k_m2_residual, dim3(G, B), dim3(256), 0, st, V, 0);
        }
        return hipGetLastError();
    }

    hipError_t launch_m2_iteration(hipStream_t st, DevView const& V, int mode, double t, double last_step, bool do_factor, hipEvent_t ev0, hipEvent_t ev1,
                                   int stamp_mode, bool companion, double companion_dt)
    {
        return V.high_occupancy ? m2_sequence<4>(st, V, mode, t, last_step, do_factor, ev0, ev1, false, stamp_mode, companion, companion_dt)
                                : m2_sequence<2>(st, V, mode, t, last_step, do_factor, ev0, ev1, false, stamp_mode, companion, companion_dt);
    }

    hipError_t launch_m2_refine(hipStream_t st, DevView const& V)
    {
        int const B = V.batch, G = grid_per_instance(V);
        hipLaunchKernelGGL(k_m2_residual, dim3(G, B), dim3(256), 0, st, V, 1);
        DevView Vr = V;
        Vr.rhs = V.rres;
        hipError_t const e = V.high_occupancy ? m2_sequence<4>(st, Vr, 0, 0.0, 0.0, true, nullptr, nullptr, true) : m2_sequence<2>(st, Vr, 0, 0.0, 0.0, true, nullptr, nullptr, true);
        if(e != hipSuccess) return e;
        hipLaunchKernelGGL(k_m2_refine_apply, dim3(G, B), dim3(256), 0, st, V);
        hipLaunchKernelGGL(k_m2_clear_eta, dim3((B + 63) / 64), dim3(64), 0, st, V);
        hipLaunchKernelGGL(k_m2_residual, dim3(G, B), dim3(256), 0, st, V, 0);
        hipLaunchKernelGGL(k_m2_retest, dim3(G, B), dim3(256), 0, st, V);
        return hipGetLastError();
    }

    __global__ void __launch_bounds__(256) k_m2_publish(int const* __restrict__ flags, double const* __restrict__ eta, int batch, int* pub_flags, double* pub_eta,
                                                        unsigned long long* pub_seq, unsigned long long seq)
    {
        for(int b = static_cast<int>(threadIdx.x); b < batch; b += static_cast<int>(blockDim.x)) pub_flags[b] = flags[b];
        if(eta)
            for(int i = static_cast<int>(threadIdx.x); i < 4 * batch; i += static_cast<int>(blockDim.x)) pub_eta[i] = eta[i];
        __threadfence_system();
        __syncthreads();
        if(threadIdx.x == 0) __hip_atomic_store(pub_seq, seq, __ATOMIC_RELEASE, __HIP_MEMORY_SCOPE_SYSTEM);
    }
    hipError_t launch_m2_publish(hipStream_t st, DevView const& V, int* pub_flags, double* pub_eta, unsigned long long* pub_seq, unsigned long long seq)
    {
        hipLaunchKernelGGL(k_m2_publish, dim3(1), dim3(256), 0, st, V.flags, V.residual_tol > 0.0 ? V.eta_acc : nullptr, V.batch, pub_flags, pub_eta, pub_seq, seq);
        return hipGetLastError();
    }

    struct M2GraphEntry
    {
        hipGraph_t graph{};
        hipGraphExec_t exec{};
        hipGraphNode_t eval_node{}, publish_node{};
        DevView V{};
        int mode{}, do_factor{}, dyn{}, companion{};
        int* pub_flags{};
        double* pub_eta{};
        unsigned long long* pub_seq{};
    };
    struct M2GraphCache
    {
        std::vector<M2GraphEntry> entries;
        ~M2GraphCache() { clear(); }
        void clear()
        {
            for(auto& e: entries)
            {
                if(e.exec) (void)hipGraphExecDestroy(e.exec);
                if(e.graph) (void)hipGraphDestroy(e.graph);
            }
            entries.clear();
        }
    };
    M2GraphCache* m2_graphs_create() { return new M2GraphCache; }
    void m2_graphs_destroy(M2GraphCache* c) { delete c; }
    void m2_graphs_clear(M2GraphCache* c)
    {
        if(c) c->clear();
    }

    hipError_t launch_m2_iteration_graph(hipStream_t st, M2GraphCache* cache, DevView const& V, int mode, double t, double last_step, bool do_factor, int stamp_mode,
                                         bool companion, double companion_dt, int* pub_flags, double* pub_eta, unsigned long long* pub_seq, unsigned long long seq)
    {
        int const dyn = (V.dyn_a && V.dyn_b) ? stamp_mode : 0;
        M2GraphEntry* hit = nullptr;
        for(auto& e: cache->entries)
            if(e.mode == mode && e.do_factor == (do_factor ? 1 : 0) && e.dyn == dyn && e.companion == (companion ? 1 : 0) && e.pub_flags == pub_flags && e.pub_eta == pub_eta &&
               e.pub_seq == pub_seq && std::memcmp(&e.V, &V, sizeof(DevView)) == 0)
            {
                hit = &e;
                break;
            }
        if(!hit)
        {
            if(cache->entries.size() >= 16) cache->clear();
            M2GraphEntry e;
            std::memcpy(&e.V, &V, sizeof(DevView));
            e.mode = mode;
            e.do_factor = do_factor ? 1 : 0;
            e.dyn = dyn;
            e.companion = companion ? 1 : 0;
            e.pub_flags = pub_flags;
            e.pub_eta = pub_eta;
            e.pub_seq = pub_seq;
            hipError_t rc = hipStreamBeginCapture(st, hipStreamCaptureModeRelaxed);
            if(rc != hipSuccess) return rc;
            rc = V.high_occupancy ? m2_sequence<4>(st, V, mode, t, last_step, do_factor, nullptr, nullptr, false, stamp_mode, companion, companion_dt)
                                  : m2_sequence<2>(st, V, mode, t, last_step, do_factor, nullptr, nullptr, false, stamp_mode, companion, companion_dt);
            hipError_t const rp = launch_m2_publish(st, V, pub_flags, pub_eta, pub_seq, seq);
            hipError_t const re = hipStreamEndCapture(st, &e.graph);
            if(rc != hipSuccess) return rc;
            if(rp != hipSuccess) return rp;
            if(re != hipSuccess) return re;
            rc = hipGraphInstantiate(&e.exec, e.graph, nullptr, nullptr, 0);
            if(rc != hipSuccess)
            {
                (void)hipGraphDestroy(e.graph);
                return rc;
            }
            size_t n = 0;
            rc = hipGraphGetNodes(e.graph, nullptr, &n);
            if(rc != hipSuccess) return rc;
            std::vector<hipGraphNode_t> nodes(n);
            rc = hipGraphGetNodes(e.graph, nodes.data(), &n);
            if(rc != hipSuccess) return rc;
            for(hipGraphNode_t nd: nodes)
            {
                hipGraphNodeType ty{};
                if(hipGraphNodeGetType(nd, &ty) != hipSuccess || ty != hipGraphNodeTypeKernel) continue;
                hipKernelNodeParams kp{};
                if(hipGraphKernelNodeGetParams(nd, &kp) != hipSuccess) continue;
                if(kp.func == reinterpret_cast<void*>(&k_m2_eval)) e.eval_node = nd;
                else if(kp.func == reinterpret_cast<void*>(&k_m2_publish))
                    e.publish_node = nd;
            }
            if(!e.eval_node || !e.publish_node)
            {
                (void)hipGraphExecDestroy(e.exec);
                (void)hipGraphDestroy(e.graph);
                return hipErrorInvalidValue;
            }
            cache->entries.push_back(e);
            hit = &cache->entries.back();
        }
        {
            DevView v = V;
            int md = mode, dy = dyn == 1 ? 1 : 0, cs = companion ? 1 : 0;
            double tt = t, ls = last_step, cd = companion_dt;
            void* args[] = {&v, &md, &tt, &ls, &dy, &cs, &cd};
            hipKernelNodeParams kp{};
            hipError_t rc = hipGraphKernelNodeGetParams(hit->eval_node, &kp);
            if(rc != hipSuccess) return rc;
            kp.kernelParams = args;
            kp.extra = nullptr;
            rc = hipGraphExecKernelNodeSetParams(hit->exec, hit->eval_node, &kp);
            if(rc != hipSuccess) return rc;
        }
        {
            int const* fl = V.flags;
            double const* eta = V.residual_tol > 0.0 ? V.eta_acc : nullptr;
            int batch = V.batch;
// ... 524 lines not shown
```

### phy-engine_amd/csrc/pe_kernels.hpp

```cpp
#pragma once
#include <hip/hip_runtime_api.h>

#include <cstddef>

#include "pe_device.hpp"

#ifndef PE_THREADS
    #define PE_THREADS 512
#endif

namespace pe
{
    hipError_t launch_tr_steps(hipStream_t st, DevView const& V, double dt, int nsteps, bool reuse_factor);
    hipError_t launch_dc_point(hipStream_t st, DevView const& V, int mode);
    hipError_t launch_factor_solve(hipStream_t st, DevView const& V, bool do_factor);
    hipError_t launch_m2_companion(hipStream_t st, DevView const& V, double dt);
    hipError_t launch_m2_iteration(hipStream_t st, DevView const& V, int mode, double t, double last_step, bool do_factor, hipEvent_t ev0 = nullptr,
                                   hipEvent_t ev1 = nullptr, int stamp_mode = 0, bool companion = false, double companion_dt = 0.0);
    struct M2GraphCache;
    M2GraphCache* m2_graphs_create();
    void m2_graphs_destroy(M2GraphCache* c);
    void m2_graphs_clear(M2GraphCache* c);
    hipError_t launch_m2_iteration_graph(hipStream_t st, M2GraphCache* cache, DevView const& V, int mode, double t, double last_step, bool do_factor, int stamp_mode,
                                         bool companion, double companion_dt, int* pub_flags, double* pub_eta, unsigned long long* pub_seq, unsigned long long seq);
    hipError_t launch_stream_copy(hipStream_t st, void const* src, void* dst, size_t bytes);
    hipError_t launch_m2_refine(hipStream_t st, DevView const& V);
    hipError_t launch_m2_publish(hipStream_t st, DevView const& V, int* pub_flags, double* pub_eta, unsigned long long* pub_seq, unsigned long long seq);
    hipError_t launch_ac_residual(hipStream_t st, DevView const& V, double const* xacc, double const* b0, int rhs0, double* worst);
    hipError_t launch_ac_accumulate(hipStream_t st, DevView const& V, double* xacc, double* b0, bool first);
    hipError_t launch_csr_residual(hipStream_t st, DevView const& V, double const* xacc, double const* b0, double* worst);
    hipError_t launch_sweep_statistics(hipStream_t st, DevView const& V, int n_chunks, double* partial, double* out);
    hipError_t launch_probe_arm(hipStream_t st, ProbedView const& V);
    hipError_t launch_probe_record(hipStream_t st, ProbedView const& V, double t);
    struct AcSweepView;
    hipError_t launch_ac_sweep_fill(hipStream_t st, DevView const& V, AcSweepView const& S);
    hipError_t launch_ac_residual_each(hipStream_t st, DevView const& V, AcSweepView const& S);
    hipError_t launch_ac_accumulate_each(hipStream_t st, DevView const& V, AcSweepView const& S, bool first);
    hipError_t launch_ac_sweep_gather(hipStream_t st, DevView const& V, AcSweepView const& S);
    struct NoiseView;
    hipError_t launch_noise_sources(hipStream_t st, DevView const& V, NoiseView const& Z);
    hipError_t launch_noise_accumulate(hipStream_t st, DevView const& V, NoiseView const& Z);
    struct LteView;
    struct StateCopy;
    hipError_t launch_tr_lte(hipStream_t st, DevView const& V, LteView const& L);
    hipError_t launch_tr_history_push(hipStream_t st, DevView const& V, double* hist, int slot);
    hipError_t launch_tr_state_copy(hipStream_t st, StateCopy const& S);
    struct DcSweepView;
    hipError_t launch_dc_sweep_fill(hipStream_t st, DevView const& V, DcSweepView const& S);
    hipError_t launch_dc_sweep_seed(hipStream_t st, DevView const& V, DcSweepView const& S, bool from_main);
    hipError_t launch_dc_sweep_classify(hipStream_t st, DevView const& V, DcSweepView const& S, bool reseed);
    hipError_t launch_dc_sweep_gather(hipStream_t st, DevView const& V, DcSweepView const& S);
}
```

### phy-engine_amd/csrc/pe_quad.hpp

```cpp
#pragma once
#include "pe_device.hpp"

#ifndef PE_QUAD_LDS_STACK
    #define PE_QUAD_LDS_STACK 0
#endif
#ifndef PE_QUAD_BACK_LAZY_FENCE
    #define PE_QUAD_BACK_LAZY_FENCE 1
#endif
#ifndef PE_QUAD_ELIM_GUARD
    #define PE_QUAD_ELIM_GUARD 1
#endif
#ifndef PE_QUAD_COLS
    #define PE_QUAD_COLS 8
#endif
#if defined(__HIPCC__)
    #define PEQ_DEV __device__ __forceinline__
#else
    #define PEQ_DEV inline
#endif

namespace pe
{
    template <class X>
    struct QuadCtx
// ... 583 lines not shown
            for(int s2 = 0; s2 < RS; ++s2)
            {
                vi const R = r + 16 * s2;
                vu const so = cx.offR + (X::to_u(R - p) << 3) + static_cast<unsigned>(sptr) * 8u;
                X::when(cx.valid & (R >= p) & (R < m), [&] { X::st(cx.baseR, so + static_cast<unsigned>(u) * ub, g[s2]); });
            }
            X::when(cx.valid & (r < p), [&] { X::st(cx.baseW, cx.offW + static_cast<unsigned>(c0) * 8u + (X::to_u(r) << 3), g[0]); });
        }
        if constexpr(RS > 1)
        {
#pragma unroll
            for(int kk = 0; kk < 16; ++kk) a[0][kk] = X::sel(r > kk, a[0][kk], vd(0.0));
            quad_chunks<X, RS, 16>(V, cx, blk, L, m, p, nch, lptr, sptr, a);
        }
        return bad;
    }

    template <class X>
    PEQ_DEV void quad_factor_list(DevView const& V, int quad, int list)
    {
        using vi = typename X::vi;
        using vu = typename X::vu;
        using vm = typename X::vm;
        int const* ql = V.q_list + static_cast<long long>(quad) * 4;
        int const b0 = ql[0];
        if(b0 < 0) return;
        vi const lane = X::lane();
        vi const q = lane >> 4;
        vi const b = X::ld_i32(ql, X::to_u(q) << 2);
        QuadCtx<X> cx;
        cx.valid = b >= 0;
        vi const bb = X::sel(cx.valid, b, vi(b0));
        vu const d = X::to_u(bb - b0);
        cx.r = lane & 15;
        cx.offA = d * static_cast<unsigned>(V.nnzA * 8ll);
        cx.offF = d * static_cast<unsigned>(V.factor_doubles * 8ll);
        cx.offR = d * static_cast<unsigned>(V.arena_doubles * 8ll);
        cx.offW = d * static_cast<unsigned>(V.rows * 8ll);
        cx.baseA = reinterpret_cast<char const*>(V.aval + static_cast<long long>(b0) * V.nnzA);
        cx.baseF = reinterpret_cast<char*>(V.factor + static_cast<long long>(b0) * V.factor_doubles);
        cx.baseR = reinterpret_cast<char*>(V.arena + static_cast<long long>(b0) * V.arena_doubles);
        cx.baseW = reinterpret_cast<char*>(V.w + static_cast<long long>(b0) * V.rows);
        cx.ldsq = X::to_u(q) * static_cast<unsigned>(V.q_lds_stride * 8) + 8u;
        cx.ldsz = X::to_u(q) * static_cast<unsigned>(V.q_lds_stride * 8);
#if PE_QUAD_LDS_STACK
        if(V.q_lds_stride > 0)
        {
            X::when(cx.r == 0, [&] { X::lds_st(cx.ldsz, typename X::vd(0.0)); });
            X::lds_fence();
        }
#endif
        int const* lp = V.q_lists + 2 * list;
        int const* blk = V.q_prog + lp[0];
        int const nfr = lp[1];
        vm bad = X::none();
        long long clkv[6] = {0, 0, 0, 0, 0, 0};
        bool const clk = V.prof && list == 0 && (V.quad & 32);
        if(nfr > 0)
        {
            QuadLaneIdx<X> cur;
            quad_lane_idx<X>(cur, V.q_lane + blk[10], blk[5], cx.r);
            for(int i = 0; i < nfr; ++i)
            {
                int const rs = blk[5], nch = blk[4], rs_next = blk[11];
                QuadLaneIdx<X> nxt;
                quad_lane_idx<X>(nxt, V.q_lane + (rs_next ? blk[12] : blk[10]), rs_next ? rs_next : rs, cx.r);
                if(rs == 1) bad = bad | quad_front<X, 1>(V, cx, blk, cur, clk, clkv);
                else
                    bad = bad | quad_front<X, 2>(V, cx, blk, cur, clk, clkv);
                cur = nxt;
                blk += 16 + 32 * nch;
            }
        }
        if(clk) X::prof(V.prof + static_cast<long long>(b0) * PE_PROF + 64, clkv, 6);
        X::flag(V.flags, bb, 4, bad & cx.valid & (cx.r == 0));
    }

    template <class X>
    PEQ_DEV void quad_factor_mid_list(DevView const& V, int quad, int list)
    {
        using vi = typename X::vi;
        using vu = typename X::vu;
        using vm = typename X::vm;
        int const* lp = V.q2_lists + 2 * list;
        int const nfr = lp[1];
        if(nfr <= 0) return;
        int const* ql = V.q_list + static_cast<long long>(quad) * 4;
        int const b0 = ql[0];
        if(b0 < 0) return;
        vi const lane = X::lane();
        vi const q = lane >> 4;
        vi const b = X::ld_i32(ql, X::to_u(q) << 2);
        QuadCtx<X> cx;
        cx.valid = b >= 0;
        vi const bb = X::sel(cx.valid, b, vi(b0));
        vu const d = X::to_u(bb - b0);
        cx.r = lane & 15;
        cx.offA = d * static_cast<unsigned>(V.nnzA * 8ll);
        cx.offF = d * static_cast<unsigned>(V.factor_doubles * 8ll);
        cx.offR = d * static_cast<unsigned>(V.arena_doubles * 8ll);
        cx.offW = d * static_cast<unsigned>(V.rows * 8ll);
        cx.baseA = reinterpret_cast<char const*>(V.aval + static_cast<long long>(b0) * V.nnzA);
        cx.baseF = reinterpret_cast<char*>(V.factor + static_cast<long long>(b0) * V.factor_doubles);
        cx.baseR = reinterpret_cast<char*>(V.arena + static_cast<long long>(b0) * V.arena_doubles);
        cx.baseW = reinterpret_cast<char*>(V.w + static_cast<long long>(b0) * V.rows);
        cx.ldsq = vu(0u);
// ... 151 lines not shown
```

### phy-engine_amd/csrc/pe_symbolic.cpp

```cpp
#include "pe_symbolic.hpp"

#include <algorithm>
#include <cmath>
#include <numeric>

namespace pe
{
    namespace
    {
        using ivec = std::vector<int>;

        bool match_rows(int n, int const* rp, int const* ci, double const* vals, double diag_rel, ivec& rmatch, int& swaps)
        {
            rmatch.assign(n, -1);
            ivec colof(n, -1);
            std::vector<double> rowmax(n, 0.0);
            for(int i = 0; i < n; ++i)
                for(int e = rp[i]; e < rp[i + 1]; ++e) rowmax[i] = std::max(rowmax[i], vals ? std::fabs(vals[e]) : 1.0);
            for(int i = 0; i < n; ++i)
            {
                for(int e = rp[i]; e < rp[i + 1]; ++e)
                {
                    if(ci[e] != i) continue;
                    double const w = vals ? std::fabs(vals[e]) : 1.0;
// ... 652 lines not shown
                        if(l < 0)
                        {
                            S.error = "internal: child update row missing from parent front";
                            return false;
                        }
                        S.f_rel[a] = l;
                    }
                }
                S.tree_depth = std::max(S.tree_depth, depth[s]);
            }
        }

        S.col_src = q;
        S.row_src.resize(n);
        for(int k = 0; k < n; ++k) S.row_src[k] = rmatch[q[k]];

        {
            ivec qinv(n), eq2k(n);
            for(int k = 0; k < n; ++k) qinv[q[k]] = k;
            for(int k = 0; k < n; ++k) eq2k[S.row_src[k]] = k;
            S.f_asm_ptr.assign(nf + 1, 0);
            int const nnz = rp[n];
            ivec owner(nnz), pos(nnz);
            for(int i = 0; i < n; ++i)
            {
                int const k = eq2k[i];
                for(int e = rp[i]; e < rp[i + 1]; ++e)
                {
                    int const l = qinv[ci[e]];
                    int const s = col2front[std::min(k, l)];
                    int const r = local_of(s, k), c = local_of(s, l);
                    if(r < 0 || c < 0)
                    {
                        S.error = "internal: matrix entry outside its front";
                        return false;
                    }
                    owner[e] = s;
                    pos[e] = (r << 16) | c;
                    ++S.f_asm_ptr[s + 1];
                }
            }
            for(int s = 0; s < nf; ++s) S.f_asm_ptr[s + 1] += S.f_asm_ptr[s];
            S.asm_slot.resize(nnz);
            S.asm_pos.resize(nnz);
            ivec fill(S.f_asm_ptr.begin(), S.f_asm_ptr.end() - 1);
            for(int e = 0; e < nnz; ++e)
            {
                int const d = fill[owner[e]]++;
                S.asm_slot[d] = e;
                S.asm_pos[d] = pos[e];
            }
        }

        int const W = std::max(1, opt.n_waves);
        int const K = std::max(1, opt.n_parts);
        S.n_parts = K;
        S.f_kind.assign(nf, 1);
        ivec part_of(nf, K > 1 ? -1 : 0);
        std::vector<double> cost(nf, 0.0), sub(nf, 0.0);
        std::vector<char> fits(nf, 1), fits_mid(nf, opt.quad_mid ? 1 : 0), fits_quad(nf, opt.quad ? 1 : 0);
        double total = 0.0;
        for(int s = 0; s < nf; ++s)
        {
            double const m = S.f_p[s] + S.f_u[s];
            cost[s] = 400.0 + m * m * (2.0 + S.f_p[s]);
            total += cost[s];
            fits[s] = fits[s] && m <= opt.wave_m && S.f_p[s] <= opt.wave_p;
            fits_quad[s] = fits_quad[s] && m <= 32 && S.f_p[s] <= 16 && S.f_asm_ptr[s + 1] - S.f_asm_ptr[s] <= 255 && S.f_child_ptr[s + 1] - S.f_child_ptr[s] <= 16;
            if(fits[s] && opt.wave_slot > 0)
            {
                long long const mm = S.f_p[s] + S.f_u[s], whole = (pe_ld(static_cast<int>(mm)) + 1LL) * mm,
                                panel = static_cast<long long>(pe_ld(static_cast<int>(mm))) * S.f_p[s] + static_cast<long long>(pe_ld(S.f_p[s])) * S.f_u[s] + mm;
                if(whole > opt.wave_slot && panel > opt.wave_slot) fits[s] = 0;
            }
            fits_mid[s] = fits_mid[s] && m <= 64 && S.f_p[s] <= 16 && S.f_asm_ptr[s + 1] - S.f_asm_ptr[s] <= 255 && S.f_child_ptr[s + 1] - S.f_child_ptr[s] <= 16;
            sub[s] += cost[s];
            int const P = S.f_parent[s];
            if(P >= 0)
            {
                sub[P] += sub[s];
                if(!fits[s]) fits[P] = 0;
                if(!fits_mid[s]) fits_mid[P] = 0;
                if(!fits_quad[s]) fits_quad[P] = 0;
            }
        }
        auto mark_subtree = [&](int root, auto&& fn)
        {
            ivec st2{root};
            while(!st2.empty())
            {
                int const t = st2.back();
                st2.pop_back();
                fn(t);
                for(int a = S.f_child_ptr[t]; a < S.f_child_ptr[t + 1]; ++a) st2.push_back(S.f_child[a]);
            }
        };
        std::vector<double> part_total(K, 0.0);
        if(K > 1)
        {
            double const limit1 = total / (static_cast<double>(K) * opt.part_cut);
            ivec stack, sroots;
            for(int s = 0; s < nf; ++s)
                if(S.f_parent[s] < 0) stack.push_back(s);
            while(!stack.empty())
            {
                int const s = stack.back();
// ... 101 lines not shown
            std::vector<ivec> lists(static_cast<size_t>(K) * (W + 1));
            for(int s = 0; s < nf; ++s)
                if(exec_of[s] >= 0) lists[exec_of[s]].push_back(s);
            S.wave_ptr.assign(static_cast<size_t>(K) * (W + 1) + 1, 0);
            S.wave_list.clear();
            S.coop_ptr.assign(K + 1, 0);
            S.coop_list.clear();
            for(int q = 0; q < K; ++q)
            {
                for(int w = 0; w <= W; ++w)
                {
                    size_t const e = static_cast<size_t>(q) * (W + 1) + w;
                    if(w < W) S.wave_list.insert(S.wave_list.end(), lists[e].begin(), lists[e].end());
                    S.wave_ptr[e + 1] = static_cast<int>(S.wave_list.size());
                }
                auto const& cl = lists[static_cast<size_t>(q) * (W + 1) + W];
                S.coop_list.insert(S.coop_list.end(), cl.begin(), cl.end());
                S.coop_ptr[q + 1] = static_cast<int>(S.coop_list.size());
            }
            ivec h(nf, 0);
            int maxh = 0;
            for(int s = 0; s < nf; ++s)
            {
                if(S.f_kind[s] != 2) continue;
                int hh = 1;
                for(int a = S.f_child_ptr[s]; a < S.f_child_ptr[s + 1]; ++a)
                    if(S.f_kind[S.f_child[a]] == 2) hh = std::max(hh, h[S.f_child[a]] + 1);
                h[s] = hh;
                maxh = std::max(maxh, hh);
            }
            S.top_ptr.assign(maxh + 1, 0);
            S.top_list.clear();
            for(int lev = 1; lev <= maxh; ++lev)
            {
                for(int s = 0; s < nf; ++s)
                    if(S.f_kind[s] == 2 && h[s] == lev) S.top_list.push_back(s);
                S.top_ptr[lev] = static_cast<int>(S.top_list.size());
            }

            S.f_lptr.resize(nf);
            S.f_uptr.resize(nf);
            S.f_sptr.assign(nf, 0);
            long long fo = 0;
            for(int s = 0; s < nf; ++s)
            {
                long long const p = S.f_p[s], u = S.f_u[s], m = p + u;
                S.f_lptr[s] = fo;
                fo += m * p;
                S.f_uptr[s] = fo;
                fo += p * u;
            }
            S.factor_doubles = fo;
            long long base = 0;
            auto persistent = [&](int s)
            {
                int const P = S.f_parent[s];
                return exec_of[s] < 0 || P < 0 || exec_of[P] != exec_of[s] || S.f_kind[s] == 3 || (S.f_quad[s] && !S.f_quad[P]);
            };
            for(int s = 0; s < nf; ++s)
                if(persistent(s))
                {
                    S.f_sptr[s] = base;
                    base += static_cast<long long>(S.f_u[s]) * (S.f_u[s] + 1);
                }
            for(auto const& lst: lists)
            {
                long long sp[2] = {0, 0}, peak[2] = {0, 0};
                std::vector<long long> rel_off(lst.size(), 0);
                for(size_t qi = 0; qi < lst.size(); ++qi)
                {
                    int const s = lst[qi];
                    for(int a = S.f_child_ptr[s]; a < S.f_child_ptr[s + 1]; ++a)
                    {
                        int const c = S.f_child[a];
                        if(!persistent(c)) sp[depth[c] & 1] -= static_cast<long long>(S.f_u[c]) * (S.f_u[c] + 1);
                    }
                    if(persistent(s)) continue;
                    int const q = depth[s] & 1;
                    rel_off[qi] = sp[q];
                    sp[q] += static_cast<long long>(S.f_u[s]) * (S.f_u[s] + 1);
                    peak[q] = std::max(peak[q], sp[q]);
                }
                if(sp[0] != 0 || sp[1] != 0)
                {
                    S.error = "internal: executor stacks not empty at the end";
                    return false;
                }
                for(size_t qi = 0; qi < lst.size(); ++qi)
                {
                    int const s = lst[qi];
                    if(!persistent(s)) S.f_sptr[s] = base + ((depth[s] & 1) ? peak[0] : 0) + rel_off[qi];
                }
                base += peak[0] + peak[1];
            }
            S.work_doubles = 0;
            if(opt.quad)
            {
                S.q_zero_off = base;
                base += Symbolic::Q_ZERO;
            }
            S.arena_doubles = base;
        }
        S.f_inv_off.assign(S.f_child.size(), -1);
        S.f_cnp.assign(S.f_child.size(), 0);
        S.f_bmask.assign(S.f_child.size(), 0u);
        S.f_inv.clear();
        S.wave_panel_doubles = 1;
        for(int s = 0; s < nf; ++s)
        {
            int const m = S.f_p[s] + S.f_u[s];
            if(S.f_kind[s] == 0) S.wave_panel_doubles = std::max<long long>(S.wave_panel_doubles, static_cast<long long>(pe_ld(m)) * S.f_p[s] + static_cast<long long>(pe_ld(S.f_p[s])) * S.f_u[s]);
// ... 63 lines not shown
                    bool const same_list = P >= 0 && std::find(lst.begin(), lst.end(), P) != lst.end();
                    if(lds_doubles > 0) S.q_lds_total += need;
                    if(same_list && need > 0 && top + need <= lds_doubles)
                    {
                        lds_off[s] = top;
                        top += need;
                        S.q_lds_kept += need;
                    }
                    q[13] = lds_off[s];
                }
                if(i > 0)
                {
                    prog[prev_hdr + 11] = rs;
                    prog[prev_hdr + 12] = static_cast<int>(l0);
                }
                prev_hdr = h;
                for(int e = S.f_asm_ptr[s]; e < S.f_asm_ptr[s + 1]; ++e)
                {
                    int const r = S.asm_pos[e] >> 16, c = S.asm_pos[e] & 0xffff;
                    lane[l0 + static_cast<size_t>(r) * rec + c] = static_cast<unsigned char>(1 + (e - S.f_asm_ptr[s]));
                }
                for(int a = 0; a < nch; ++a)
                {
                    int const c = S.f_child[ch0 + a];
                    int* cb = q + Symbolic::Q_HDR + a * Symbolic::Q_CHILD;
                    cb[0] = static_cast<int>(S.f_sptr[c]);
                    cb[1] = S.f_u[c];
                    cb[18] = lds_off[c];
                    unsigned char* cm = reinterpret_cast<unsigned char*>(cb + 2);
                    for(int k = 0; k < S.f_u[c]; ++k)
                    {
                        int const l = S.f_rel[S.f_rows_ptr[c] + k];
                        cm[l] = static_cast<unsigned char>(1 + k);
                        lane[l0 + static_cast<size_t>(l) * rec + M + a] = static_cast<unsigned char>(1 + k);
                    }
                }
            }
        }
        lane.resize(lane.size() + 64, 0);
    }

    void build_quad_plan(Symbolic& S, int lds_doubles)
    {
        S.quad = 1;
        S.q_lds_doubles = std::max(0, lds_doubles);
        S.q_lds_kept = S.q_lds_total = 0;
        int const K = std::max(1, S.n_parts), W = static_cast<int>((S.wave_ptr.size() - 1) / K) - 1;
        std::vector<std::vector<int>> lists(static_cast<size_t>(K) * W);
        for(int part = 0; part < K; ++part)
            for(int w = 0; w < W; ++w)
                for(int i = S.wave_ptr[part * (W + 1) + w]; i < S.wave_ptr[part * (W + 1) + w + 1]; ++i)
                    if(S.f_quad[S.wave_list[i]]) lists[static_cast<size_t>(part) * W + w].push_back(S.wave_list[i]);
        build_quad_program(S, lists, S.q_lds_doubles, S.q_prog, S.q_lists, S.q_lane);
        S.q_bprog.clear();
        std::vector<int> col_owner(static_cast<size_t>(S.n), -1);
        for(int s = 0; s < S.nfronts; ++s)
            for(int c = 0; c < S.f_p[s]; ++c) col_owner[static_cast<size_t>(S.f_col0[s] + c)] = s;
        std::vector<char> pending(static_cast<size_t>(S.nfronts), 0);
        for(auto const& lst: lists)
        {
            std::vector<int> since_fence;
            for(auto it = lst.rbegin(); it != lst.rend(); ++it)
            {
                int const s = *it;
                bool need = it == lst.rbegin();
                for(int j = 0; j < S.f_u[s] && !need; ++j)
                {
                    int const o = col_owner[static_cast<size_t>(S.f_rows[S.f_rows_ptr[s] + j])];
                    need = o >= 0 && pending[static_cast<size_t>(o)];
                }
                if(need)
                {
                    for(int t: since_fence) pending[static_cast<size_t>(t)] = 0;
                    since_fence.clear();
                }
                pending[static_cast<size_t>(s)] = 1;
                since_fence.push_back(s);
                size_t const h = S.q_bprog.size();
                S.q_bprog.resize(h + Symbolic::Q_BACK, 0);
                int* q = S.q_bprog.data() + h;
                q[0] = S.f_p[s] + S.f_u[s];
                q[1] = S.f_p[s];
                q[2] = S.f_col0[s];
                q[3] = S.f_u[s];
                q[4] = static_cast<int>(S.f_lptr[s] & 0xffffffffll);
                q[5] = static_cast<int>(S.f_lptr[s] >> 32);
                q[6] = need ? 1 : 0;
                for(int j = 0; j < S.f_u[s]; ++j) q[8 + j] = S.f_rows[S.f_rows_ptr[s] + j];
            }
            for(int t: since_fence) pending[static_cast<size_t>(t)] = 0;
        }
        S.n_mid = 0;
        std::vector<std::vector<int>> mlists(static_cast<size_t>(K) * W);
        for(int part = 0; part < K; ++part)
        {
            std::vector<int> roots, root_of(S.nfronts, -1);
            std::vector<double> cost(S.nfronts, 0.0);
            for(int i = S.coop_ptr[part + 1] - 1; i >= S.coop_ptr[part]; --i)
            {
                int const s = S.coop_list[i];
                if(S.f_kind[s] != 3) continue;
                ++S.n_mid;
                int const P = S.f_parent[s];
                root_of[s] = (P >= 0 && S.f_kind[P] == 3) ? root_of[P] : s;
                if(root_of[s] == s) roots.push_back(s);
                double const m = S.f_p[s] + S.f_u[s];
// ... 149 lines not shown
```

### phy-engine_amd/csrc/pe_symbolic.hpp

```cpp
#pragma once
#include <cstdint>
#include <string>
#include <vector>

namespace pe
{
    constexpr int pe_ld(int n) { return n | 1; }
    constexpr long long front_lds_need(int mode, int p, int u)
    {
        long long const m = p + u;
        if(mode == 3) return 0;
        return (mode == 0 ? static_cast<long long>(pe_ld(p + u)) * m : static_cast<long long>(pe_ld(p + u)) * p + static_cast<long long>(pe_ld(p)) * u) + m;
    }

    struct SymbolicOptions
    {
        int nd_leaf{24};
        int relax_small{8};
        double relax_zero_frac{0.30};
        int max_pivots{48};
        double match_diag_rel{1e-8};
        int wave_m{48};
        int wave_p{24};
        long long wave_slot{0};
        int absorb_m{48};
        int n_waves{8};
        double cut_factor{1.0};
        int n_parts{1};
        double part_cut{1.5};
        int shared_cu{};
        int quad{};
        int quad_mid{};
        int quad_lds_doubles{};
        std::vector<char> const* big_unknowns{nullptr};
        int max_pivots_top{64};
        long long panel_doubles_top{0};
        long long panel_doubles_mid{0};
    long long panel_reserve{384};
    long long panel_doubles{18000};
    };

    struct Symbolic
    {
        int n{};
        int nnzA{};
        std::vector<int> row_src, col_src;

        int nfronts{};
        std::vector<int> f_col0;
        std::vector<int> f_p;
        std::vector<int> f_u;
        std::vector<int> f_parent;
        std::vector<int> f_rows_ptr;
        std::vector<int> f_rows;
        std::vector<int> f_child_ptr, f_child;
        std::vector<int> f_rel_ptr, f_rel;
        std::vector<int> f_asm_ptr;
        std::vector<int> asm_slot;
        std::vector<int> asm_pos;
        std::vector<long long> f_lptr;
        std::vector<long long> f_uptr;
        std::vector<long long> f_sptr;
        long long factor_doubles{};
        long long arena_doubles{};
        long long work_doubles{};
        long long wave_panel_doubles{};
        std::vector<int> f_kind;
        std::vector<int> f_quad;
        std::vector<int> f_wstack, f_wpar;
        int wave_stack{1};
        int n_parts{1};
        std::vector<int> wave_ptr, wave_list;
        std::vector<int> coop_ptr, coop_list;
        std::vector<int> top_ptr, top_list;
        std::vector<long long> f_inv_off;
        std::vector<int> f_cnp;
        std::vector<int> f_inv;
        std::vector<unsigned> f_bmask;
        int max_m{};
        int max_u{};

        std::vector<int> f_mode;
        std::vector<int> f_keep;
        std::vector<int> gl_ptr, gl_rptr;
        std::vector<long long> gl_sptr;
        std::vector<unsigned short> gl_dst;
        std::vector<int> gl_cnt, gl_src;

        enum : int
        {
            Q_HDR = 16,
            Q_CHILD = 32,
            Q_ZERO = 4224
        };
        int quad{};
        int q_lds_doubles{};
        long long q_lds_kept{}, q_lds_total{};
        std::vector<int> q_prog, q_lists;
        std::vector<unsigned char> q_lane;
        enum : int
        {
            Q_BACK = 40
        };
        std::vector<int> q_bprog;
        std::vector<int> q2_prog, q2_lists;
        std::vector<unsigned char> q2_lane;
        int n_mid{};
        long long q_zero_off{};

        long long nnz_LU{};
        long long nnz_LU_stored{};
        double flops{};
        int tree_depth{};
        int n_row_swaps{};
        bool structurally_singular{};
        std::string error;
    };

    bool analyze(int n, int const* rp, int const* ci, double const* vals, SymbolicOptions const& opt, Symbolic& out);

    bool build_assembly_lists(Symbolic& S, long long cap_wave, long long cap_team, int const* top_wide = nullptr, long long cap_top = 0, long long cap_mid = 0);
}
```

### phy-engine_amd/ffi.py

```python
from __future__ import annotations

import ctypes as C
import os

import numpy as np

_HERE = os.path.dirname(os.path.abspath(__file__))
LIB_PATH = os.environ.get("PE_HIP_LIB", os.path.join(_HERE, "libpe_hip.so"))

R, CAP, L, VDC, VAC, IDC, DIODE = 1, 2, 3, 4, 5, 6, 7
IAC, VCCS, VCVS, CCCS, CCVS, OPAMP, XFMR, SWITCH, VGEN, COUPLED_L = 8, 9, 10, 11, 12, 13, 14, 15, 16, 17
NMOS, PMOS, BJT_NPN, BJT_PNP, RELAY, XFMR_CT = 18, 19, 20, 21, 22, 23
DIODE_NPARAM = 11
MODE_OP, MODE_DC, MODE_TR, MODE_TROP = 0, 1, 4, 5
OK, ERR_ARG, ERR_NO_DEVICE, ERR_SINGULAR, ERR_NO_CONVERGENCE, ERR_INTERNAL, ERR_INACCURATE = 0, -1, -2, -3, -4, -5, -6

EXPORTS = [
    "pe_hip_device_count", "pe_hip_create", "pe_hip_destroy", "pe_hip_last_error", "pe_hip_solve_csr_real", "pe_hip_solve_csr_complex", "pe_hip_build_id",
    "pe_hip_load_circuit", "pe_hip_set_options", "pe_hip_get_info", "pe_hip_get_front_table", "pe_hip_set_digital_drives", "pe_hip_set_overlay", "pe_hip_set_knob", "pe_hip_get_knob", "pe_hip_update_param",
    "pe_hip_reset", "pe_hip_analyze_dc", "pe_hip_analyze_tr", "pe_hip_get_solution", "pe_hip_set_solution",
    "pe_hip_get_instance_state", "pe_hip_sweep_statistics", "pe_hip_measure_hbm_ceiling", "pe_hip_get_safety_net_counters", "pe_hip_get_newton_trace", "pe_hip_get_matrix", "pe_hip_analyze_pattern",
    "pe_hip_analyze_pattern_fronts", "pe_hip_get_phase_clocks", "pe_hip_get_phase_clocks_ex", "pe_hip_analyze_ac", "pe_hip_get_solution_ac", "pe_hip_set_ac_sweep_rows", "pe_hip_analyze_ac_sweep", "pe_hip_get_ac_sweep", "pe_hip_checkpoint_size", "pe_hip_checkpoint_save", "pe_hip_checkpoint_load", "pe_hip_set_time",
    "pe_hip_sweep_create", "pe_hip_sweep_destroy", "pe_hip_sweep_last_error", "pe_hip_sweep_devices", "pe_hip_sweep_shard", "pe_hip_sweep_set_options",
    "pe_hip_sweep_load_circuit", "pe_hip_sweep_reset", "pe_hip_sweep_operating_point", "pe_hip_sweep_run", "pe_hip_sweep_reduce", "pe_hip_sweep_get_solution",
    "pe_hip_sweep_get_instance_state", "pe_hip_set_probes", "pe_hip_arm_probes", "pe_hip_get_probe_samples", "pe_hip_get_measures",
    "pe_hip_sweep_set_probes", "pe_hip_sweep_arm_probes", "pe_hip_sweep_get_probe_samples", "pe_hip_sweep_get_measures",
    "pe_hip_analyze_tr_adaptive", "pe_hip_get_tr_step_log",
    "pe_hip_analyze_noise", "pe_hip_get_noise", "pe_hip_get_noise_sources", "pe_hip_get_noise_source_density", "pe_hip_get_noise_integrated",
    "pe_hip_set_dc_sweep_rows", "pe_hip_analyze_dc_sweep", "pe_hip_get_dc_sweep", "pe_hip_get_dc_sweep_status",
]
DC_SWEEP_PARALLEL, DC_SWEEP_TRACE = 0, 1
MEAS_MIN, MEAS_MAX, MEAS_AVG, MEAS_RMS, MEAS_INTEG, MEAS_CROSS = 1, 2, 3, 4, 5, 6
_MEAS_NAMES = {"min": MEAS_MIN, "max": MEAS_MAX, "avg": MEAS_AVG, "rms": MEAS_RMS, "integ": MEAS_INTEG, "cross": MEAS_CROSS}


class DeviceTable(C.Structure):
    _fields_ = [("kind", C.c_int), ("count", C.c_int), ("nodes", C.POINTER(C.c_int)), ("branch", C.POINTER(C.c_int)),
                ("params", C.POINTER(C.c_double)), ("params_batched", C.c_int)]


class Options(C.Structure):
    _fields_ = [("v_abstol", C.c_double), ("v_reltol", C.c_double), ("i_abstol", C.c_double), ("i_reltol", C.c_double),
                ("g_min", C.c_double), ("max_newton", C.c_int), ("refactor_every_solve", C.c_int), ("r_open", C.c_double), ("residual_tol", C.c_double)]


class Timings(C.Structure):
    _fields_ = [(n, C.c_double) for n in ("h2d_ms", "solve_ms", "d2h_ms", "solve_host_ms", "total_host_ms", "analyze_ms")]


class Info(C.Structure):
    _fields_ = [("rows", C.c_int), ("n_nodes", C.c_int), ("n_branches", C.c_int), ("batch", C.c_int), ("nnz_a", C.c_int),
                ("nnz_lu", C.c_longlong), ("nnz_lu_stored", C.c_longlong), ("n_fronts", C.c_int), ("max_front", C.c_int),
                ("tree_depth", C.c_int), ("n_row_swaps", C.c_int), ("factor_flops", C.c_double),
                ("bytes_per_instance", C.c_longlong), ("n_r", C.c_int), ("n_c", C.c_int), ("n_l", C.c_int), ("n_v", C.c_int),
                ("n_i", C.c_int), ("n_d", C.c_int), ("nonlinear", C.c_int), ("n_parts", C.c_int), ("n_top_levels", C.c_int),
                ("n_wavefronts", C.c_int), ("lds_bytes", C.c_int), ("nnz_lu_stored_top", C.c_longlong), ("n_wave_fronts", C.c_int),
                ("n_quad_fronts", C.c_int), ("nnz_lu_stored_quad", C.c_longlong), ("mid_top_limit", C.c_int), ("ew_grid", C.c_int),
                ("quad_lds_pad", C.c_int)]

    def asdict(self):
        return {k: getattr(self, k) for k, _ in self._fields_}


class Measure(C.Structure):
    _fields_ = [("kind", C.c_int), ("probe", C.c_int), ("edge", C.c_int), ("occurrence", C.c_int), ("level", C.c_double)]


def _measures(measures):
    ms = list(measures)
    arr = (Measure * max(1, len(ms)))()
    for i, m in enumerate(ms):
        if isinstance(m, dict):
            kind, probe = m["kind"], m["probe"]
            level, edge, occ = m.get("level", 0.0), m.get("edge", 0), m.get("occurrence", 1)
        else:
            kind, probe = m[0], m[1]
            level = m[2] if len(m) > 2 else 0.0
            edge = m[3] if len(m) > 3 else 0
            occ = m[4] if len(m) > 4 else 1
        kind = _MEAS_NAMES.get(kind, kind) if isinstance(kind, str) else kind
        arr[i] = Measure(int(kind), int(probe), int(edge), int(occ), float(level))
    return len(ms), arr
# ... 64 lines not shown


class AcSweepStats(C.Structure):
    _fields_ = [("n_points", C.c_int), ("n_passes", C.c_int), ("points_per_pass", C.c_int), ("n_analyses", C.c_int), ("n_refine_rounds", C.c_int),
                ("n_fallback_points", C.c_int), ("gpu_ms", C.c_double)]

    def asdict(self):
        return {k: getattr(self, k) for k, _ in self._fields_}


class DcSweepControl(C.Structure):
    _fields_ = [("kind", C.c_int), ("index", C.c_int), ("column", C.c_int), ("mode", C.c_int), ("order", C.c_int), ("continuation", C.c_int),
                ("max_rounds", C.c_int)]


class DcSweepStats(C.Structure):
    _fields_ = [("n_points", C.c_int), ("n_passes", C.c_int), ("points_per_pass", C.c_int), ("n_rounds", C.c_int), ("n_failed_cold", C.c_longlong),
                ("n_reseeded", C.c_longlong), ("n_failed", C.c_longlong), ("newton_iters", C.c_longlong), ("n_analyses", C.c_int), ("gpu_ms", C.c_double)]

    def asdict(self):
        return {k: getattr(self, k) for k, _ in self._fields_}


class NoiseControl(C.Structure):
    _fields_ = [("out_pos", C.c_int), ("out_neg", C.c_int), ("temp_k", C.c_double), ("keep_contributions", C.c_int)]


class NoiseStats(C.Structure):
    _fields_ = [("n_points", C.c_int), ("n_sources", C.c_int), ("n_passes", C.c_int), ("points_per_pass", C.c_int), ("n_analyses", C.c_int),
                ("n_refine_rounds", C.c_int), ("n_retried_points", C.c_int), ("gpu_ms", C.c_double)]

    def asdict(self):
        return {k: getattr(self, k) for k, _ in self._fields_}


_lib = None


def lib():
    global _lib
    if _lib is None:
        if not os.path.exists(LIB_PATH):
            raise RuntimeError(f"{LIB_PATH} not built: run `make -C phy-engine_amd/csrc` (or __graft_entry__.build())")
        l = C.CDLL(LIB_PATH)
        l.pe_hip_last_error.restype = C.c_char_p
        l.pe_hip_last_error.argtypes = [C.c_void_p]
        l.pe_hip_create.argtypes = [C.c_int, C.POINTER(C.c_void_p)]
        l.pe_hip_destroy.argtypes = [C.c_void_p]
        l.pe_hip_destroy.restype = None
        l.pe_hip_load_circuit.argtypes = [C.c_void_p, C.c_int, C.c_int, C.c_int, C.c_int, C.POINTER(DeviceTable)]
        l.pe_hip_set_options.argtypes = [C.c_void_p, C.POINTER(Options)]
        l.pe_hip_get_info.argtypes = [C.c_void_p, C.POINTER(Info)]
        l.pe_hip_get_front_table.argtypes = [C.c_void_p, C.c_int, C.c_int] + [C.POINTER(C.c_int)] * 9
        l.pe_hip_set_digital_drives.argtypes = [C.c_void_p, C.c_int, C.POINTER(C.c_int), C.POINTER(C.c_double)]
        l.pe_hip_update_param.argtypes = [C.c_void_p, C.c_int, C.c_int, C.c_int, C.POINTER(C.c_double), C.c_int]
        l.pe_hip_reset.argtypes = [C.c_void_p]
        l.pe_hip_analyze_dc.argtypes = [C.c_void_p, C.c_int, C.POINTER(RunStats)]
        l.pe_hip_analyze_tr.argtypes = [C.c_void_p, C.c_double, C.c_int, C.POINTER(RunStats)]
        l.pe_hip_get_solution.argtypes = [C.c_void_p, C.c_int, C.c_int, C.POINTER(C.c_double)]
        l.pe_hip_set_solution.argtypes = [C.c_void_p, C.c_int, C.c_int, C.POINTER(C.c_double)]
        l.pe_hip_sweep_statistics.argtypes = [C.c_void_p, C.POINTER(C.c_double)]
        l.pe_hip_get_safety_net_counters.argtypes = [C.c_void_p, C.POINTER(C.c_longlong), C.POINTER(C.c_longlong), C.POINTER(C.c_int)]
        l.pe_hip_measure_hbm_ceiling.argtypes = [C.c_void_p, C.c_size_t, C.c_int, C.POINTER(C.c_double)]
        l.pe_hip_get_instance_state.argtypes = [C.c_void_p, C.c_int, C.c_int, C.POINTER(C.c_int), C.POINTER(C.c_longlong),
                                                C.POINTER(C.c_longlong), C.POINTER(C.c_double)]
        l.pe_hip_get_newton_trace.argtypes = [C.c_void_p, C.c_int, C.POINTER(C.c_int), C.POINTER(C.c_int)]
        l.pe_hip_get_matrix.argtypes = [C.c_void_p, C.c_int, C.POINTER(C.c_int), C.POINTER(C.c_int), C.POINTER(C.c_double),
                                        C.POINTER(C.c_double)]
        l.pe_hip_solve_csr_real.argtypes = [C.c_void_p, C.c_int, C.c_int, C.POINTER(C.c_int), C.POINTER(C.c_int),
                                            C.POINTER(C.c_double), C.POINTER(C.c_double), C.POINTER(C.c_double), C.c_int,
                                            C.POINTER(Timings)]
        l.pe_hip_solve_csr_complex.argtypes = l.pe_hip_solve_csr_real.argtypes
        l.pe_hip_build_id.restype = C.c_char_p
        l.pe_hip_build_id.argtypes = []
        l.pe_hip_analyze_pattern.argtypes = [C.c_int, C.POINTER(C.c_int), C.POINTER(C.c_int), C.POINTER(C.c_double), C.POINTER(Info)]
        _probe_argtypes(l, "pe_hip_")
        _probe_argtypes(l, "pe_hip_sweep_")
        l.pe_hip_set_ac_sweep_rows.argtypes = [C.c_void_p, C.c_int, C.POINTER(C.c_int)]
        l.pe_hip_analyze_ac_sweep.argtypes = [C.c_void_p, C.c_int, C.POINTER(C.c_double), C.POINTER(C.c_int), C.POINTER(AcSweepStats)]
        l.pe_hip_get_ac_sweep.argtypes = [C.c_void_p, C.c_int, C.c_int, C.c_int, C.c_int, C.POINTER(C.c_double), C.POINTER(C.c_double)]
        l.pe_hip_analyze_noise.argtypes = [C.c_void_p, C.c_int, C.POINTER(C.c_double), C.POINTER(NoiseControl), C.POINTER(C.c_int), C.POINTER(NoiseStats)]
        l.pe_hip_get_noise.argtypes = [C.c_void_p, C.c_int, C.c_int, C.c_int, C.c_int, C.POINTER(C.c_double), C.POINTER(C.c_double)]
        l.pe_hip_get_noise_sources.argtypes = [C.c_void_p, C.c_int] + [C.POINTER(C.c_int)] * 6
        l.pe_hip_get_noise_source_density.argtypes = [C.c_void_p, C.c_int, C.c_int, C.POINTER(C.c_double)]
        l.pe_hip_get_noise_integrated.argtypes = [C.c_void_p, C.c_int, C.c_int, C.POINTER(C.c_double)]
        l.pe_hip_set_dc_sweep_rows.argtypes = [C.c_void_p, C.c_int, C.POINTER(C.c_int)]
        l.pe_hip_analyze_dc_sweep.argtypes = [C.c_void_p, C.c_int, C.POINTER(C.c_double), C.POINTER(DcSweepControl), C.POINTER(C.c_int), C.POINTER(DcSweepStats)]
        l.pe_hip_get_dc_sweep.argtypes = [C.c_void_p, C.c_int, C.c_int, C.c_int, C.c_int, C.POINTER(C.c_double)]
        l.pe_hip_get_dc_sweep_status.argtypes = [C.c_void_p, C.c_int, C.c_int, C.c_int, C.c_int] + [C.POINTER(C.c_int)] * 3
        l.pe_hip_analyze_tr_adaptive.argtypes = [C.c_void_p, C.c_double, C.POINTER(TrControl), C.POINTER(TrAdaptiveStats)]
        l.pe_hip_get_tr_step_log.argtypes = [C.c_void_p, C.c_longlong, C.c_int, C.POINTER(C.c_double), C.POINTER(C.c_int), C.POINTER(C.c_longlong)]
        _lib = l
    return _lib


def _ip(a):
    return a.ctypes.data_as(C.POINTER(C.c_int))


def _dp(a):
    return a.ctypes.data_as(C.POINTER(C.c_double))


class PeHipError(RuntimeError):
    def __init__(self, code, msg):
        super().__init__(f"pe_hip error {code}: {msg}")
# ... 100 lines not shown
            pass

    def _chk(self, rc, allow=()):
        if rc != 0 and rc not in allow:
            raise PeHipError(rc, lib().pe_hip_last_error(self._h).decode())
        return rc

    def set_options(self, g_min=0.0, v_abstol=0.0, v_reltol=0.0, i_abstol=0.0, i_reltol=0.0, max_newton=0, refactor_every_solve=1, r_open=0.0, residual_tol=0.0):
        o = Options(v_abstol, v_reltol, i_abstol, i_reltol, g_min, max_newton, refactor_every_solve, r_open, residual_tol)
        self._chk(lib().pe_hip_set_options(self._h, C.byref(o)))

    def set_knob(self, name, value):
        self._chk(lib().pe_hip_set_knob(self._h, name.encode(), int(value)))

    def get_knob(self, name):
        v, s = C.c_int(0), C.c_int(0)
        self._chk(lib().pe_hip_get_knob(self._h, name.encode(), C.byref(v), C.byref(s)))
        return v.value if s.value else None

    def set_digital_drives(self, nodes, volts):
        n = np.ascontiguousarray(nodes, dtype=np.int32)
        v = np.ascontiguousarray(volts, dtype=np.float64)
        self._chk(lib().pe_hip_set_digital_drives(self._h, len(n), _ip(n), _dp(v)))

    def load(self, n_nodes, n_branches, tables, batch=1):
        arr = (DeviceTable * max(1, len(tables)))()
        self._keep = list(tables)
        for i, (kind, nodes, branch, par, batched) in enumerate(tables):
            arr[i] = DeviceTable(kind, len(nodes), _ip(nodes), None if branch is None else _ip(branch), _dp(par), batched)
        self._chk(lib().pe_hip_load_circuit(self._h, int(n_nodes), int(n_branches), int(batch), len(tables), arr))
        self.rows = n_nodes + n_branches
        self.batch = batch
        self._probe_cfg = (0, 0, 0)
        self._ac_rows = None
        self._dc_rows = None

    def load_deck(self, deck, batch=1, overrides=None, n_drives=0):
        n_nodes, n_br, tables = deck_tables(deck, batch, overrides, n_drives)
        self.load(n_nodes, n_br, tables, batch)

    def info(self):
        i = Info()
        self._chk(lib().pe_hip_get_info(self._h, C.byref(i)))
        return i.asdict()

    def front_table(self, which=0):
        n = C.c_int()
        self._chk(lib().pe_hip_get_front_table(self._h, int(which), 0, *[None] * 8, C.byref(n)))
        names = ("p", "u", "parent", "kind", "quad", "mode", "n_children", "n_own")
        out = {k: np.zeros(n.value, dtype=np.int32) for k in names}
        self._chk(lib().pe_hip_get_front_table(self._h, int(which), n.value, *[_ip(out[k]) for k in names], C.byref(n)))
        return out

    def reset(self):
        self._chk(lib().pe_hip_reset(self._h))

    def analyze_tr(self, dt, nsteps, check=True):
        st = RunStats()
        rc = lib().pe_hip_analyze_tr(self._h, float(dt), int(nsteps), C.byref(st))
        if check:
            self._chk(rc)
        d = st.asdict()
        d["rc"] = rc
        return d

    def analyze_tr_adaptive(self, t_stop, dt_init, dt_min=0.0, dt_max=0.0, lte_reltol=0.0, lte_abstol_v=0.0, lte_abstol_i=0.0, trtol=0.0,
                            max_steps=0, source_breakpoints=False, breakpoints=(), check=True):
        bp = np.ascontiguousarray(breakpoints, dtype=np.float64).reshape(-1)
        c = TrControl(float(dt_init), float(dt_min), float(dt_max), float(lte_reltol), float(lte_abstol_v), float(lte_abstol_i), float(trtol),
                      int(max_steps), 1 if source_breakpoints else 0, len(bp), _dp(bp) if len(bp) else None)
        st = TrAdaptiveStats()
        rc = lib().pe_hip_analyze_tr_adaptive(self._h, float(t_stop), C.byref(c), C.byref(st))
        if check:
            self._chk(rc)
        d = st.asdict()
        d["rc"] = rc
        return d

    def tr_step_log(self):
        n = C.c_longlong(0)
        self._chk(lib().pe_hip_get_tr_step_log(self._h, 0, 0, None, None, C.byref(n)))
        dt = np.empty(n.value)
        oc = np.empty(n.value, dtype=np.int32)
        if n.value:
            self._chk(lib().pe_hip_get_tr_step_log(self._h, 0, int(n.value), _dp(dt), _ip(oc), C.byref(n)))
        return dt, oc

    def analyze_dc(self, mode=MODE_DC, check=True):
        st = RunStats()
        rc = lib().pe_hip_analyze_dc(self._h, int(mode), C.byref(st))
        if check:
            self._chk(rc)
        d = st.asdict()
        d["rc"] = rc
        return d

    def solution(self, first=0, count=None):
        count = self.batch - first if count is None else count
        x = np.empty((count, self.rows))
        self._chk(lib().pe_hip_get_solution(self._h, first, count, _dp(x)))
        return x

    def safety_net(self):
        a, b, c = C.c_longlong(0), C.c_longlong(0), C.c_int(0)
        self._chk(lib().pe_hip_get_safety_net_counters(self._h, C.byref(a), C.byref(b), C.byref(c)))
        return {"refined": a.value, "rematched": b.value, "careful": bool(c.value)}
# ... 284 lines not shown
```

Measured before the change: 54840.

## Skip refactoring static elimination-tree fronts on later Newton iterations

Marks fronts whose assembled entries and pivot rows don't depend on nonlinear devices as static. It builds a reduced lane-group program that contains only the dynamic fronts, and keeps the Schur contributions of static subtree roots in persistent arena slots. From the second Newton iteration on, the factorization runs only the dynamic fronts. This needs extra arena memory, saved results, and stats counters, and it is gated to nonlinear circuits with no overlay and no refinement.

```diff
diff --git a/include/pe_hip.h b/include/pe_hip.h
--- a/include/pe_hip.h
+++ b/include/pe_hip.h
@@ -135,6 +135,9 @@
 int pe_hip_get_info(pe_hip_engine* h, pe_hip_info* out);
 int pe_hip_get_front_table(pe_hip_engine* h, int which, int capacity, int* pivots, int* updates, int* parent, int* kind, int* quad, int* mode,
                            int* n_children, int* n_own, int* n_fronts);
+int pe_hip_get_static_fronts(pe_hip_engine* h, int which, int capacity, int* is_static, int* n_fronts);
+int pe_hip_get_static_skip_stats(pe_hip_engine* h, long long* skipped_launches, long long* full_launches);
+int pe_hip_get_static_skip_refinement_stats(pe_hip_engine* h, long long* launches_after_refinement, long long* skipped_after_refinement);
 
 int pe_hip_set_knob(pe_hip_engine* h, const char* name, int value);
 int pe_hip_get_knob(pe_hip_engine* h, const char* name, int* value, int* is_set);
diff --git a/phy-engine_amd/csrc/pe_device.hpp b/phy-engine_amd/csrc/pe_device.hpp
--- a/phy-engine_amd/csrc/pe_device.hpp
+++ b/phy-engine_amd/csrc/pe_device.hpp
@@ -177,6 +177,25 @@
     };
     static_assert(offsetof(DevView, v_abstol) == offsetof(DevView, probe_armed) + sizeof(int), "probe_armed must fill the padding before v_abstol");
 
+    struct StaticSkip
+    {
+        int const *q_prog_dyn{}, *q_lists_dyn{};
+        unsigned char const* row_keep{};
+        double* wy{};
+        int save{}, skip{};
+    };
+    inline StaticSkip static_skip_effective(DevView const& V, bool do_factor, int stamp_mode, bool refine, StaticSkip const* sk)
+    {
+        StaticSkip eff = sk ? *sk : StaticSkip{};
+        bool const have_lists = V.dyn_a && V.dyn_b;
+        eff.skip = (sk && sk->skip && !refine && do_factor && stamp_mode == 1 && have_lists && V.quad && V.n_mid == 0 && V.q_lds_stride == 0) ? 1 : 0;
+        eff.save = (sk && sk->save && !eff.skip && !refine && do_factor && V.quad && V.n_quads > 0) ? 1 : 0;
+        return eff;
+    }
+#if !defined(__HIPCC__)
+    inline thread_local StaticSkip const* host_static_skip = nullptr;
+#endif
+
     struct ProbedView : DevView
     {
         ProbeView pr{};
diff --git a/phy-engine_amd/csrc/pe_engine.cpp b/phy-engine_amd/csrc/pe_engine.cpp
--- a/phy-engine_amd/csrc/pe_engine.cpp
+++ b/phy-engine_amd/csrc/pe_engine.cpp
@@ -452,6 +452,9 @@
     h->sym_dt = 0.0;
     h->careful = false;
     h->n_refined = h->n_rematched = 0;
+    h->quad_skipped_launches = h->quad_full_launches = 0;
+    h->quad_launches_after_refinement = h->quad_skipped_after_refinement = 0;
+    h->static_skip = pe::StaticSkip{};
     h->sym_pool.release();
     ac_sweep_drop(h);
     dc_sweep_drop(h);
@@ -538,6 +541,35 @@
         if(n_children) n_children[s] = S->f_child_ptr[s + 1] - S->f_child_ptr[s];
         if(n_own) n_own[s] = S->f_asm_ptr[s + 1] - S->f_asm_ptr[s];
     }
+    return PE_HIP_OK;
+}
+
+int pe_hip_get_static_fronts(pe_hip_engine* h, int which, int capacity, int* is_static, int* n_fronts)
+{
+    if(!h || !n_fronts || capacity < 0) return PE_HIP_ERR_ARG;
+    pe::Symbolic const* S = nullptr;
+    if(which == 0 && h->loaded && h->sym_class >= 0) S = &h->sym;
+    else if(which == 1 && h->csr.have) S = &h->csr.sym;
+    else if(which == 2 && h->csrz.have) S = &h->csrz.sym;
+    if(!S) return fail(h, PE_HIP_ERR_ARG, "get_static_fronts: no such analysis");
+    *n_fronts = S->nfronts;
+    for(int s = 0; s < S->nfronts && s < capacity && is_static; ++s) is_static[s] = static_cast<size_t>(s) < S->f_static.size() ? S->f_static[static_cast<size_t>(s)] : 0;
+    return PE_HIP_OK;
+}
+
+int pe_hip_get_static_skip_stats(pe_hip_engine* h, long long* skipped_launches, long long* full_launches)
+{
+    if(!h) return PE_HIP_ERR_ARG;
+    if(skipped_launches) *skipped_launches = h->quad_skipped_launches;
+    if(full_launches) *full_launches = h->quad_full_launches;
+    return PE_HIP_OK;
+}
+
+int pe_hip_get_static_skip_refinement_stats(pe_hip_engine* h, long long* launches_after_refinement, long long* skipped_after_refinement)
+{
+    if(!h) return PE_HIP_ERR_ARG;
+    if(launches_after_refinement) *launches_after_refinement = h->quad_launches_after_refinement;
+    if(skipped_after_refinement) *skipped_after_refinement = h->quad_skipped_after_refinement;
     return PE_HIP_OK;
 }
 
diff --git a/phy-engine_amd/csrc/pe_engine_internal.hpp b/phy-engine_amd/csrc/pe_engine_internal.hpp
--- a/phy-engine_amd/csrc/pe_engine_internal.hpp
+++ b/phy-engine_amd/csrc/pe_engine_internal.hpp
@@ -149,6 +149,10 @@
     std::vector<char> a_static;
     double a_static_dt{-1.0};
     double analyze_ms{};
+    pe::StaticSkip static_skip{};
+    long long quad_skipped_launches{}, quad_full_launches{};
+    long long quad_launches_after_refinement{}, quad_skipped_after_refinement{};
+    bool refined_in_point{};
 
     struct Ac
     {
@@ -290,7 +294,7 @@
     int upload_symbolic(pe_hip_engine* h, Pool& pool, pe::Symbolic& S, pe::SymbolicOptions const& so, pe::DevView& V, int batch);
     pe::SymbolicOptions symbolic_options(pe_hip_engine const* h, int batch_in, int rows, int panel_reserve = 384, int force_resident = 0);
     int analyze_fitting(pe_hip_engine* h, int batch, int geometry_rows, int n, int const* rp, int const* ci, double const* vals, pe::Symbolic& S,
-                        pe::SymbolicOptions& so);
+                        pe::SymbolicOptions& so, std::vector<char> const* dyn_slots = nullptr, std::vector<char> const* dyn_rows = nullptr);
     int ensure_symbolic(pe_hip_engine* h, bool tr, double dt);
     pe::ProbedView probe_view(pe_hip_engine const* h);
     void probe_disarm(pe_hip_engine* h);
diff --git a/phy-engine_amd/csrc/pe_engine_newton.cpp b/phy-engine_amd/csrc/pe_engine_newton.cpp
--- a/phy-engine_amd/csrc/pe_engine_newton.cpp
+++ b/phy-engine_amd/csrc/pe_engine_newton.cpp
@@ -241,6 +241,8 @@
             for(int b: todo) mask[b] = 1;
             if(int const urc = upload_active(h, mask); urc != PE_HIP_OK) return urc;
             HIPCHK(h, pe::launch_m2_refine(h->stream, h->V));
+            h->refined_in_point = true;
+            if(h->V.quad && h->V.n_quads > 0) ++h->quad_full_launches;
             HIPCHK(h, hipStreamSynchronize(h->stream));
             if(int const rc = pull_eta(); rc != PE_HIP_OK) return rc;
             std::vector<int> fl(B);
@@ -285,6 +287,9 @@
             h->active_dev.clear();
         }
         if(graph_mode && !h->graphs) h->graphs = pe::m2_graphs_create();
+        h->refined_in_point = false;
+        bool const may_skip_static = h->static_skip.q_prog_dyn && h->hc.nonlinear && do_factor && !has_overlay(h) && h->V.quad && h->V.n_mid == 0 &&
+                                     h->V.q_lds_stride == 0 && h->V.dyn_a && h->V.dyn_b && knob(h, "STATIC_SKIP", 1) != 0;
         for(int it = 0; it < max_it && n_active > 0; ++it)
         {
             if(has_overlay(h))
@@ -293,21 +298,33 @@
             static bool const full_stamp = env_int0("PHY_ENGINE_HIP_FULL_STAMP", 0) != 0;
             int const dyn = full_stamp ? 0 : (it > 0 ? 1 : (a_static_ok ? 2 : 0));
             bool const comp = it == 0 && companion_dt != nullptr;
+            pe::StaticSkip sk = h->static_skip;
+            sk.save = (may_skip_static && !full_stamp && it == 0) ? 1 : 0;
+            sk.skip = (may_skip_static && !full_stamp && it > 0 && dyn == 1 && !h->refined_in_point) ? 1 : 0;
+            if(do_factor && h->V.quad && h->V.n_quads > 0)
+            {
+                ++(sk.skip ? h->quad_skipped_launches : h->quad_full_launches);
+                if(it > 0 && h->refined_in_point)
+                {
+                    ++h->quad_launches_after_refinement;
+                    if(sk.skip) ++h->quad_skipped_after_refinement;
+                }
+            }
             std::vector<double> eta_now;
             if(graph_mode)
             {
                 if(int const prc = ensure_published(h, static_cast<size_t>(B)); prc != PE_HIP_OK) return prc;
                 auto const dev = pub_view(h->pub_dev, static_cast<size_t>(B));
                 unsigned long long const seq = ++h->pub_seq;
-                HIPCHK(h, pe::launch_m2_iteration_graph(h->stream, h->graphs, h->V, mode, t, last_step, do_factor, dyn, comp, companion_dt ? *companion_dt : 0.0, dev.flags,
-                                                        dev.eta, dev.seq, seq));
+                HIPCHK(h, pe::launch_m2_iteration_graph_static(h->stream, h->graphs, h->V, mode, t, last_step, do_factor, dyn, comp, companion_dt ? *companion_dt : 0.0,
+                                                               dev.flags, dev.eta, dev.seq, seq, sk));
                 ++launches;
                 if(int const prc = wait_published(h, S.flags, &eta_now, seq); prc != PE_HIP_OK) return prc;
             }
             else
             {
-                HIPCHK(h, pe::launch_m2_iteration(h->stream, h->V, mode, t, last_step, do_factor, h->evk0, h->evk1, dyn, comp,
-                                                  companion_dt ? *companion_dt : 0.0));
+                HIPCHK(h, pe::launch_m2_iteration_static(h->stream, h->V, mode, t, last_step, do_factor, h->evk0, h->evk1, dyn, comp,
+                                                         companion_dt ? *companion_dt : 0.0, sk));
                 ++launches;
                 if(use_publish)
                 {
@@ -542,6 +559,31 @@
             int size() const { return 1; }
             void sync() const {}
         };
+    }
+    namespace
+    {
+        struct HostStaticSkip
+        {
+            StaticSkip eff;
+            HostStaticSkip(DevView const& V, bool do_factor, int stamp_mode, StaticSkip const& sk) : eff(static_skip_effective(V, do_factor, stamp_mode, false, &sk))
+            {
+                host_static_skip = (eff.skip || eff.save) ? &eff : nullptr;
+            }
+            ~HostStaticSkip() { host_static_skip = nullptr; }
+        };
+    }
+    hipError_t launch_m2_iteration_static(hipStream_t st, DevView const& V, int mode, double t, double last_step, bool do_factor, hipEvent_t ev0, hipEvent_t ev1,
+                                          int stamp_mode, bool companion, double companion_dt, StaticSkip const& sk)
+    {
+        HostStaticSkip const scope(V, do_factor, stamp_mode, sk);
+        return launch_m2_iteration(st, V, mode, t, last_step, do_factor, ev0, ev1, stamp_mode, companion, companion_dt);
+    }
+    hipError_t launch_m2_iteration_graph_static(hipStream_t st, M2GraphCache* cache, DevView const& V, int mode, double t, double last_step, bool do_factor,
+                                                int stamp_mode, bool companion, double companion_dt, int* pub_flags, double* pub_eta, unsigned long long* pub_seq,
+                                                unsigned long long seq, StaticSkip const& sk)
+    {
+        HostStaticSkip const scope(V, do_factor, stamp_mode, sk);
+        return launch_m2_iteration_graph(st, cache, V, mode, t, last_step, do_factor, stamp_mode, companion, companion_dt, pub_flags, pub_eta, pub_seq, seq);
     }
     hipError_t launch_probe_arm(hipStream_t, ProbedView const& V)
     {
diff --git a/phy-engine_amd/csrc/pe_engine_policy.cpp b/phy-engine_amd/csrc/pe_engine_policy.cpp
--- a/phy-engine_amd/csrc/pe_engine_policy.cpp
+++ b/phy-engine_amd/csrc/pe_engine_policy.cpp
@@ -321,9 +321,11 @@
     }
 
     int analyze_fitting(pe_hip_engine* h, int batch, int geometry_rows, int n, int const* rp, int const* ci, double const* vals, pe::Symbolic& S,
-                        pe::SymbolicOptions& so)
+                        pe::SymbolicOptions& so, std::vector<char> const* dyn_slots, std::vector<char> const* dyn_rows)
     {
         so = symbolic_options(h, batch, geometry_rows);
+        so.dyn_slots = dyn_slots;
+        so.dyn_rows = dyn_rows;
         for(int attempt = 0;; ++attempt)
         {
             if(!pe::analyze(n, rp, ci, vals, so, S))
@@ -337,6 +339,8 @@
             }
             if(attempt == 2) return fail(h, PE_HIP_ERR_INTERNAL, "symbolic analysis: a front of order " + std::to_string(S.max_m) + " does not fit the LDS of a CU");
             so = symbolic_options(h, batch, geometry_rows, std::max(384, S.max_m + 72), attempt == 1 ? 1 : 0);
+            so.dyn_slots = dyn_slots;
+            so.dyn_rows = dyn_rows;
             if(too_deep) so.n_parts = 1;
         }
     }
@@ -355,9 +359,22 @@
             pe::estimate_values(h->hc, tr, dt, h->opt.g_min, r_open_of(h), av);
             if(char const* k = std::getenv("PHY_ENGINE_HIP_TEST_BLIND_MATCH"); k && *k == '1') std::fill(av.begin(), av.end(), 1.0);
         }
+        std::vector<char> dyn_slots, dyn_rows;
+        if(h->hc.nonlinear)
+        {
+            auto const& hc = h->hc;
+            std::vector<char> const dyn = pe::dynamic_dv_mask(hc);
+            dyn_slots.assign(hc.ci.size(), 0);
+            dyn_rows.assign(static_cast<size_t>(hc.rows), 0);
+            for(size_t e = 0; e < hc.ci.size(); ++e)
+                for(int k = hc.a_ptr[e]; k < hc.a_ptr[e + 1] && !dyn_slots[e]; ++k) dyn_slots[e] = dyn[static_cast<size_t>(hc.a_src[k] >> 1)];
+            for(int r = 0; r < hc.rows; ++r)
+                for(int k = hc.b_ptr[r]; k < hc.b_ptr[r + 1] && !dyn_rows[static_cast<size_t>(r)]; ++k) dyn_rows[static_cast<size_t>(r)] = dyn[static_cast<size_t>(hc.b_src[k] >> 1)];
+        }
         pe::SymbolicOptions so{};
         {
-            int const rc = analyze_fitting(h, h->hc.batch, h->hc.rows, h->hc.rows, h->hc.rp.data(), h->hc.ci.data(), av.data(), h->sym, so);
+            int const rc = analyze_fitting(h, h->hc.batch, h->hc.rows, h->hc.rows, h->hc.rp.data(), h->hc.ci.data(), av.data(), h->sym, so,
+                                           h->hc.nonlinear ? &dyn_slots : nullptr, h->hc.nonlinear ? &dyn_rows : nullptr);
             if(rc != PE_HIP_OK)
             {
                 h->sym_class = -1;
@@ -374,6 +391,9 @@
             if(S.quad)
                 std::fprintf(stderr, "[pe_hip]   lane-group kernel: LDS stack %d doubles per instance holds %lld of %lld update-matrix doubles of the wave fronts\n",
                              S.q_lds_doubles, S.q_lds_kept, S.q_lds_total);
+            if(S.quad)
+                std::fprintf(stderr, "[pe_hip]   lane-group kernel: %d static fronts, the persistent slots of their roots add %lld doubles to an arena of %lld\n", S.n_static_quad,
+                             S.static_root_doubles, S.arena_doubles);
             if(S.quad)
             {
                 std::fprintf(stderr, "[pe_hip]   wave-front lists (fronts):");
@@ -418,6 +438,7 @@
         }
         pe::m2_graphs_clear(h->graphs);
         h->sym_pool.release();
+        h->static_skip = pe::StaticSkip{};
         int const rc = upload_symbolic(h, h->sym_pool, h->sym, so, h->V, h->hc.batch);
         if(rc != PE_HIP_OK) return rc;
         h->active_dev.clear();
@@ -476,22 +497,11 @@
             h->V.n_dyn_a = h->V.n_dyn_b = 0;
             if(hc.nonlinear)
             {
-                std::vector<char> const dyn = pe::dynamic_dv_mask(hc);
                 std::vector<int> da, db;
                 for(size_t e = 0; e < nnz; ++e)
-                    for(int k = ptr2[e]; k < ptr2[e + 1]; ++k)
-                        if(dyn[static_cast<size_t>(src2[k] >> 1)])
-                        {
-                            da.push_back(static_cast<int>(e));
-                            break;
-                        }
+                    if(dyn_slots[static_cast<size_t>(S.asm_slot[e])]) da.push_back(static_cast<int>(e));
                 for(int r = 0; r < hc.rows; ++r)
-                    for(int k = hc.b_ptr[r]; k < hc.b_ptr[r + 1]; ++k)
-                        if(dyn[static_cast<size_t>(hc.b_src[k] >> 1)])
-                        {
-                            db.push_back(r);
-                            break;
-                        }
+                    if(dyn_rows[static_cast<size_t>(r)]) db.push_back(r);
                 h->V.n_dyn_a = static_cast<int>(da.size());
                 h->V.n_dyn_b = static_cast<int>(db.size());
                 if(da.empty()) da.push_back(0);
@@ -501,6 +511,13 @@
                 std::vector<unsigned char> rd(static_cast<size_t>(std::max(1, hc.rows)), 0);
                 for(int k = 0; k < h->V.n_dyn_b; ++k) rd[static_cast<size_t>(db[static_cast<size_t>(k)])] = 1;
                 HIPCHK(h, h->sym_pool.upload(h->V.row_dyn, rd));
+                if(S.quad && S.n_static_quad > 0)
+                {
+                    HIPCHK(h, h->sym_pool.upload(h->static_skip.q_prog_dyn, S.q_prog_dyn));
+                    HIPCHK(h, h->sym_pool.upload(h->static_skip.q_lists_dyn, S.q_lists_dyn));
+                    HIPCHK(h, h->sym_pool.upload(h->static_skip.row_keep, S.row_keep));
+                    HIPCHK(h, h->sym_pool.alloc(h->static_skip.wy, static_cast<size_t>(hc.rows) * hc.batch));
+                }
             }
             h->V.asm_slot = nullptr;
             std::vector<int> slot_e(nnz, 0);
diff --git a/phy-engine_amd/csrc/pe_front.hpp b/phy-engine_amd/csrc/pe_front.hpp
--- a/phy-engine_amd/csrc/pe_front.hpp
+++ b/phy-engine_amd/csrc/pe_front.hpp
@@ -423,10 +423,18 @@
         gather_contributions(tm.tid(), tm.size(), V.a_ptr, V.a_src, dv, V.aval + static_cast<long long>(b) * V.nnzA, 0, V.nnzA);
         gather_contributions(tm.tid(), tm.size(), V.b_ptr, V.b_src, dv, V.rhs + static_cast<long long>(b) * V.rows, 0, V.rows);
     }
-    PE_DEV void stamp_dynamic_chunk(DevView const& V, int b, int g, int G, int t0, int T, bool with_w = false, bool rhs_full = false)
+    PE_DEV void stamp_dynamic_chunk(DevView const& V, int b, int g, int G, int t0, int T, bool with_w = false, bool rhs_full = false, double const* wy = nullptr,
+                                    unsigned char const* row_keep = nullptr)
     {
         double const* dv = V.dv + static_cast<long long>(b) * V.dv_len;
         double* w = with_w ? V.w + static_cast<long long>(b) * V.rows : nullptr;
+#if !defined(__HIPCC__)
+        if(host_static_skip && host_static_skip->skip && with_w && !rhs_full)
+        {
+            wy = host_static_skip->wy;
+            row_keep = host_static_skip->row_keep;
+        }
+#endif
         auto range = [&](int n, int& lo, int& hi)
         {
             int const c = (n + G - 1) / G;
@@ -451,7 +459,7 @@
             for(int k = lo + t0; k < hi; k += T)
             {
                 int const r = V.row_src[k];
-                if(!V.row_dyn[r]) w[k] = rhs[r];
+                if(!V.row_dyn[r]) w[k] = (row_keep && row_keep[k]) ? wy[static_cast<long long>(b) * V.rows + k] : rhs[r];
             }
         }
     }
@@ -1315,6 +1323,11 @@
     PE_DEV void backward_part(Team const& tm, DevView const& V, int b, int part, double* lds)
     {
         int const* wp = V.wave_ptr + part * (V.n_waves + 1);
+#if !defined(__HIPCC__)
+        if(host_static_skip && host_static_skip->save && part == 0)
+            for(int k = 0; k < V.rows; ++k)
+                if(host_static_skip->row_keep[k]) host_static_skip->wy[static_cast<long long>(b) * V.rows + k] = V.w[static_cast<long long>(b) * V.rows + k];
+#endif
         long long const cbw0 = tm.clock();
         for(int q = V.coop_ptr[part + 1] - 1; q >= V.coop_ptr[part]; --q) front_backward(tm, V, b, V.coop_list[q], lds, V.max_m, V.lds_coop_stage);
         tm.sync();
diff --git a/phy-engine_amd/csrc/pe_kernels.hip b/phy-engine_amd/csrc/pe_kernels.hip
--- a/phy-engine_amd/csrc/pe_kernels.hip
+++ b/phy-engine_amd/csrc/pe_kernels.hip
@@ -565,11 +565,13 @@
         }
     }
 
-    __global__ void __launch_bounds__(256) k_m2_stamp(DevView V, int dynamic_only)
+    __global__ void __launch_bounds__(256) k_m2_stamp(DevView V, int dynamic_only, double const* __restrict__ wy, unsigned char const* __restrict__ row_keep)
     {
         int const b = static_cast<int>(blockIdx.y);
         if(!V.active[b]) return;
-        if(dynamic_only) stamp_dynamic_chunk(V, b, static_cast<int>(blockIdx.x), static_cast<int>(gridDim.x), static_cast<int>(threadIdx.x), static_cast<int>(blockDim.x), true, dynamic_only == 2);
+        if(dynamic_only)
+            stamp_dynamic_chunk(V, b, static_cast<int>(blockIdx.x), static_cast<int>(gridDim.x), static_cast<int>(threadIdx.x), static_cast<int>(blockDim.x), true, dynamic_only == 2, wy,
+                                row_keep);
         else
             stamp_chunk(V, b, static_cast<int>(blockIdx.x), static_cast<int>(gridDim.x), static_cast<int>(threadIdx.x), static_cast<int>(blockDim.x), true);
     }
@@ -659,6 +661,17 @@
         double const* rhs = V.rhs + static_cast<long long>(b) * V.rows;
         double* w = V.w + static_cast<long long>(b) * V.rows;
         for(int k = tm.tid(); k < V.rows; k += tm.size()) w[k] = rhs[V.row_src[k]];
+    }
+
+    __global__ void __launch_bounds__(256) k_m2_keep_y(DevView V, double* __restrict__ wy, unsigned char const* __restrict__ row_keep)
+    {
+        int const b = static_cast<int>(blockIdx.y);
+        if(!V.active[b]) return;
+        GridTeam tm;
+        double const* w = V.w + static_cast<long long>(b) * V.rows;
+        double* y = wy + static_cast<long long>(b) * V.rows;
+        for(int k = tm.tid(); k < V.rows; k += tm.size())
+            if(row_keep[k]) y[k] = w[k];
     }
 
     template <int MINW>
@@ -981,9 +994,11 @@
 
     template <int MINW>
     static hipError_t m2_sequence(hipStream_t st, DevView const& V, int mode, double t, double last_step, bool do_factor, hipEvent_t ev0, hipEvent_t ev1, bool refine,
-                                  int stamp_mode = 0, bool companion = false, double companion_dt = 0.0)
+                                  int stamp_mode = 0, bool companion = false, double companion_dt = 0.0, StaticSkip const* sk = nullptr)
     {
         bool const have_lists = V.dyn_a && V.dyn_b;
+        StaticSkip const eff = static_skip_effective(V, do_factor, stamp_mode, refine, sk);
+        bool const skip_static = eff.skip != 0, keep_y = eff.save != 0;
         int const eval_dyn = (stamp_mode == 1 && have_lists) ? 1 : 0, stamp_dyn = have_lists ? stamp_mode : 0;
         size_t const lds = static_cast<size_t>(V.lds_doubles) * sizeof(double);
         size_t const lds_s = static_cast<size_t>(V.lds_solve_doubles) * sizeof(double);
@@ -1010,7 +1025,8 @@
         if(!refine)
         {
             hipLaunchKernelGGL(k_m2_eval, dim3(G, B), dim3(256), 0, st, V, mode, t, last_step, eval_dyn, companion ? 1 : 0, companion_dt);
-            hipLaunchKernelGGL(k_m2_stamp, dim3(G, B), dim3(256), 0, st, V, stamp_dyn);
+            hipLaunchKernelGGL(k_m2_stamp, dim3(G, B), dim3(256), 0, st, V, stamp_dyn, skip_static ? static_cast<double const*>(sk->wy) : nullptr,
+                               skip_static ? sk->row_keep : nullptr);
         }
         else
             hipLaunchKernelGGL(k_m2_winit, dim3(G, B), dim3(256), 0, st, V);
@@ -1025,11 +1041,20 @@
                     hipError_t const e = set_lds(reinterpret_cast<void const*>(&k_m2_factor_quads), qlds);
                     if(e != hipSuccess) return e;
                 }
-                hipLaunchKernelGGL(k_m2_factor_quads, dim3(V.n_quads * V.n_parts * V.n_waves), dim3(64), qlds, st, V);
+                if(skip_static)
+                {
+                    DevView Vd = V;
+                    Vd.q_prog = sk->q_prog_dyn;
+                    Vd.q_lists = sk->q_lists_dyn;
+                    hipLaunchKernelGGL(k_m2_factor_quads, dim3(V.n_quads * V.n_parts * V.n_waves), dim3(64), qlds, st, Vd);
+                }
+                else
+                    hipLaunchKernelGGL(k_m2_factor_quads, dim3(V.n_quads * V.n_parts * V.n_waves), dim3(64), qlds, st, V);
                 if(V.n_mid > 0) hipLaunchKernelGGL(k_m2_factor_mid, dim3(V.n_quads * V.n_parts * V.n_waves), dim3(64), 0, st, V);
             }
             hipLaunchKernelGGL(k_m2_factor_parts<MINW>, dim3(B, V.n_parts), dim3(T), lds, st, V);
             if(ev1) (void)hipEventRecord(ev1, st);
+            if(keep_y) hipLaunchKernelGGL(k_m2_keep_y, dim3(G, B), dim3(256), 0, st, V, sk->wy, sk->row_keep);
             for_each_top_launch(V, B, MINW == 4 && T == 256, V.mid_top_limit,
                                 [&](TopLaunch const& t)
                                 {
@@ -1080,6 +1105,12 @@
         return V.high_occupancy ? m2_sequence<4>(st, V, mode, t, last_step, do_factor, ev0, ev1, false, stamp_mode, companion, companion_dt)
                                 : m2_sequence<2>(st, V, mode, t, last_step, do_factor, ev0, ev1, false, stamp_mode, companion, companion_dt);
     }
+    hipError_t launch_m2_iteration_static(hipStream_t st, DevView const& V, int mode, double t, double last_step, bool do_factor, hipEvent_t ev0, hipEvent_t ev1,
+                                          int stamp_mode, bool companion, double companion_dt, StaticSkip const& sk)
+    {
+        return V.high_occupancy ? m2_sequence<4>(st, V, mode, t, last_step, do_factor, ev0, ev1, false, stamp_mode, companion, companion_dt, &sk)
+                                : m2_sequence<2>(st, V, mode, t, last_step, do_factor, ev0, ev1, false, stamp_mode, companion, companion_dt, &sk);
+    }
 
     hipError_t launch_m2_refine(hipStream_t st, DevView const& V)
     {
@@ -1119,6 +1150,7 @@
         hipGraphNode_t eval_node{}, publish_node{};
         DevView V{};
         int mode{}, do_factor{}, dyn{}, companion{};
+        int static_bits{};
         int* pub_flags{};
         double* pub_eta{};
         unsigned long long* pub_seq{};
@@ -1144,13 +1176,29 @@
         if(c) c->clear();
     }
 
+    static hipError_t m2_iteration_graph(hipStream_t st, M2GraphCache* cache, DevView const& V, int mode, double t, double last_step, bool do_factor, int stamp_mode,
+                                         bool companion, double companion_dt, int* pub_flags, double* pub_eta, unsigned long long* pub_seq, unsigned long long seq,
+                                         StaticSkip const* sk);
     hipError_t launch_m2_iteration_graph(hipStream_t st, M2GraphCache* cache, DevView const& V, int mode, double t, double last_step, bool do_factor, int stamp_mode,
                                          bool companion, double companion_dt, int* pub_flags, double* pub_eta, unsigned long long* pub_seq, unsigned long long seq)
     {
+        return m2_iteration_graph(st, cache, V, mode, t, last_step, do_factor, stamp_mode, companion, companion_dt, pub_flags, pub_eta, pub_seq, seq, nullptr);
+    }
+    hipError_t launch_m2_iteration_graph_static(hipStream_t st, M2GraphCache* cache, DevView const& V, int mode, double t, double last_step, bool do_factor,
+                                                int stamp_mode, bool companion, double companion_dt, int* pub_flags, double* pub_eta, unsigned long long* pub_seq,
+                                                unsigned long long seq, StaticSkip const& sk)
+    {
+        return m2_iteration_graph(st, cache, V, mode, t, last_step, do_factor, stamp_mode, companion, companion_dt, pub_flags, pub_eta, pub_seq, seq, &sk);
+    }
+    static hipError_t m2_iteration_graph(hipStream_t st, M2GraphCache* cache, DevView const& V, int mode, double t, double last_step, bool do_factor, int stamp_mode,
+                                         bool companion, double companion_dt, int* pub_flags, double* pub_eta, unsigned long long* pub_seq, unsigned long long seq,
+                                         StaticSkip const* sk)
+    {
         int const dyn = (V.dyn_a && V.dyn_b) ? stamp_mode : 0;
+        int const static_bits = sk ? ((sk->save ? 1 : 0) | (sk->skip ? 2 : 0)) : 0;
         M2GraphEntry* hit = nullptr;
         for(auto& e: cache->entries)
-            if(e.mode == mode && e.do_factor == (do_factor ? 1 : 0) && e.dyn == dyn && e.companion == (companion ? 1 : 0) && e.pub_flags == pub_flags && e.pub_eta == pub_eta &&
+            if(e.mode == mode && e.do_factor == (do_factor ? 1 : 0) && e.dyn == dyn && e.companion == (companion ? 1 : 0) && e.static_bits == static_bits && e.pub_flags == pub_flags && e.pub_eta == pub_eta &&
                e.pub_seq == pub_seq && std::memcmp(&e.V, &V, sizeof(DevView)) == 0)
             {
                 hit = &e;
@@ -1165,13 +1213,14 @@
             e.do_factor = do_factor ? 1 : 0;
             e.dyn = dyn;
             e.companion = companion ? 1 : 0;
+            e.static_bits = static_bits;
             e.pub_flags = pub_flags;
             e.pub_eta = pub_eta;
             e.pub_seq = pub_seq;
             hipError_t rc = hipStreamBeginCapture(st, hipStreamCaptureModeRelaxed);
             if(rc != hipSuccess) return rc;
-            rc = V.high_occupancy ? m2_sequence<4>(st, V, mode, t, last_step, do_factor, nullptr, nullptr, false, stamp_mode, companion, companion_dt)
-                                  : m2_sequence<2>(st, V, mode, t, last_step, do_factor, nullptr, nullptr, false, stamp_mode, companion, companion_dt);
+            rc = V.high_occupancy ? m2_sequence<4>(st, V, mode, t, last_step, do_factor, nullptr, nullptr, false, stamp_mode, companion, companion_dt, sk)
+                                  : m2_sequence<2>(st, V, mode, t, last_step, do_factor, nullptr, nullptr, false, stamp_mode, companion, companion_dt, sk);
             hipError_t const rp = launch_m2_publish(st, V, pub_flags, pub_eta, pub_seq, seq);
             hipError_t const re = hipStreamEndCapture(st, &e.graph);
             if(rc != hipSuccess) return rc;
diff --git a/phy-engine_amd/csrc/pe_kernels.hpp b/phy-engine_amd/csrc/pe_kernels.hpp
--- a/phy-engine_amd/csrc/pe_kernels.hpp
+++ b/phy-engine_amd/csrc/pe_kernels.hpp
@@ -17,12 +17,17 @@
     hipError_t launch_m2_companion(hipStream_t st, DevView const& V, double dt);
     hipError_t launch_m2_iteration(hipStream_t st, DevView const& V, int mode, double t, double last_step, bool do_factor, hipEvent_t ev0 = nullptr,
                                    hipEvent_t ev1 = nullptr, int stamp_mode = 0, bool companion = false, double companion_dt = 0.0);
+    hipError_t launch_m2_iteration_static(hipStream_t st, DevView const& V, int mode, double t, double last_step, bool do_factor, hipEvent_t ev0, hipEvent_t ev1,
+                                          int stamp_mode, bool companion, double companion_dt, StaticSkip const& sk);
     struct M2GraphCache;
     M2GraphCache* m2_graphs_create();
     void m2_graphs_destroy(M2GraphCache* c);
     void m2_graphs_clear(M2GraphCache* c);
     hipError_t launch_m2_iteration_graph(hipStream_t st, M2GraphCache* cache, DevView const& V, int mode, double t, double last_step, bool do_factor, int stamp_mode,
                                          bool companion, double companion_dt, int* pub_flags, double* pub_eta, unsigned long long* pub_seq, unsigned long long seq);
+    hipError_t launch_m2_iteration_graph_static(hipStream_t st, M2GraphCache* cache, DevView const& V, int mode, double t, double last_step, bool do_factor,
+                                                int stamp_mode, bool companion, double companion_dt, int* pub_flags, double* pub_eta, unsigned long long* pub_seq,
+                                                unsigned long long seq, StaticSkip const& sk);
     hipError_t launch_stream_copy(hipStream_t st, void const* src, void* dst, size_t bytes);
     hipError_t launch_m2_refine(hipStream_t st, DevView const& V);
     hipError_t launch_m2_publish(hipStream_t st, DevView const& V, int* pub_flags, double* pub_eta, unsigned long long* pub_seq, unsigned long long seq);
diff --git a/phy-engine_amd/csrc/pe_quad.hpp b/phy-engine_amd/csrc/pe_quad.hpp
--- a/phy-engine_amd/csrc/pe_quad.hpp
+++ b/phy-engine_amd/csrc/pe_quad.hpp
@@ -659,6 +659,13 @@
 #endif
         int const* lp = V.q_lists + 2 * list;
         int const* blk = V.q_prog + lp[0];
+#if !defined(__HIPCC__)
+        if(host_static_skip && host_static_skip->skip)
+        {
+            lp = host_static_skip->q_lists_dyn + 2 * list;
+            blk = host_static_skip->q_prog_dyn + lp[0];
+        }
+#endif
         int const nfr = lp[1];
         vm bad = X::none();
         long long clkv[6] = {0, 0, 0, 0, 0, 0};
diff --git a/phy-engine_amd/csrc/pe_symbolic.cpp b/phy-engine_amd/csrc/pe_symbolic.cpp
--- a/phy-engine_amd/csrc/pe_symbolic.cpp
+++ b/phy-engine_amd/csrc/pe_symbolic.cpp
@@ -728,6 +728,19 @@
             }
         }
 
+        S.f_static.assign(nf, 0);
+        if(opt.dyn_slots && opt.dyn_rows && static_cast<int>(opt.dyn_slots->size()) == rp[n] && static_cast<int>(opt.dyn_rows->size()) == n)
+        {
+            std::vector<char> dynamic(nf, 0);
+            for(int s = 0; s < nf; ++s)
+            {
+                for(int e = S.f_asm_ptr[s]; e < S.f_asm_ptr[s + 1] && !dynamic[s]; ++e) dynamic[s] = (*opt.dyn_slots)[S.asm_slot[e]] != 0;
+                for(int k = S.f_col0[s]; k < S.f_col0[s] + S.f_p[s] && !dynamic[s]; ++k) dynamic[s] = (*opt.dyn_rows)[S.row_src[k]] != 0;
+                S.f_static[s] = dynamic[s] ? 0 : 1;
+                if(dynamic[s] && S.f_parent[s] >= 0) dynamic[S.f_parent[s]] = 1;
+            }
+        }
+
         int const W = std::max(1, opt.n_waves);
         int const K = std::max(1, opt.n_parts);
         S.n_parts = K;
@@ -935,11 +948,16 @@
             }
             S.factor_doubles = fo;
             long long base = 0;
-            auto persistent = [&](int s)
+            auto on_stacks = [&](int s)
             {
                 int const P = S.f_parent[s];
-                return exec_of[s] < 0 || P < 0 || exec_of[P] != exec_of[s] || S.f_kind[s] == 3 || (S.f_quad[s] && !S.f_quad[P]);
+                return !(exec_of[s] < 0 || P < 0 || exec_of[P] != exec_of[s] || S.f_kind[s] == 3 || (S.f_quad[s] && !S.f_quad[P]));
             };
+            auto static_quad_root = [&](int s) { return S.f_quad[s] && S.f_static[s] && S.f_parent[s] >= 0 && !S.f_static[S.f_parent[s]]; };
+            auto persistent = [&](int s) { return !on_stacks(s) || static_quad_root(s); };
+            S.static_root_doubles = 0;
+            for(int s = 0; s < nf; ++s)
+                if(on_stacks(s) && static_quad_root(s)) S.static_root_doubles += static_cast<long long>(S.f_u[s]) * (S.f_u[s] + 1);
             for(int s = 0; s < nf; ++s)
                 if(persistent(s))
                 {
@@ -1109,6 +1127,41 @@
                 for(int i = S.wave_ptr[part * (W + 1) + w]; i < S.wave_ptr[part * (W + 1) + w + 1]; ++i)
                     if(S.f_quad[S.wave_list[i]]) lists[static_cast<size_t>(part) * W + w].push_back(S.wave_list[i]);
         build_quad_program(S, lists, S.q_lds_doubles, S.q_prog, S.q_lists, S.q_lane);
+        S.n_static_quad = 0;
+        S.q_prog_dyn.clear();
+        S.q_lists_dyn.assign(2 * lists.size(), 0);
+        S.row_keep.assign(static_cast<size_t>(S.n), 0);
+        for(size_t L = 0; L < lists.size(); ++L)
+        {
+            S.q_lists_dyn[2 * L] = static_cast<int>(S.q_prog_dyn.size());
+            size_t h = static_cast<size_t>(S.q_lists[2 * L]), prev = 0;
+            int kept = 0;
+            for(int const s: lists[L])
+            {
+                size_t const len = Symbolic::Q_HDR + static_cast<size_t>(S.q_prog[h + 4]) * Symbolic::Q_CHILD;
+                if(S.f_static[s])
+                {
+                    ++S.n_static_quad;
+                    for(int k = S.f_col0[s]; k < S.f_col0[s] + S.f_p[s]; ++k) S.row_keep[static_cast<size_t>(k)] = 1;
+                }
+                else
+                {
+                    size_t const d = S.q_prog_dyn.size();
+                    S.q_prog_dyn.insert(S.q_prog_dyn.end(), S.q_prog.begin() + static_cast<long>(h), S.q_prog.begin() + static_cast<long>(h + len));
+                    S.q_prog_dyn[d + 11] = S.q_prog_dyn[d + 12] = 0;
+                    if(kept > 0)
+                    {
+                        S.q_prog_dyn[prev + 11] = S.q_prog_dyn[d + 5];
+                        S.q_prog_dyn[prev + 12] = S.q_prog_dyn[d + 10];
+                    }
+                    prev = d;
+                    ++kept;
+                }
+                h += len;
+            }
+            S.q_lists_dyn[2 * L + 1] = kept;
+        }
+        if(S.q_prog_dyn.empty()) S.q_prog_dyn.push_back(0);
         S.q_bprog.clear();
         std::vector<int> col_owner(static_cast<size_t>(S.n), -1);
         for(int s = 0; s < S.nfronts; ++s)
diff --git a/phy-engine_amd/csrc/pe_symbolic.hpp b/phy-engine_amd/csrc/pe_symbolic.hpp
--- a/phy-engine_amd/csrc/pe_symbolic.hpp
+++ b/phy-engine_amd/csrc/pe_symbolic.hpp
@@ -36,6 +36,8 @@
         int max_pivots_top{64};
         long long panel_doubles_top{0};
         long long panel_doubles_mid{0};
+        std::vector<char> const* dyn_slots{nullptr};
+        std::vector<char> const* dyn_rows{nullptr};
     long long panel_reserve{384};
     long long panel_doubles{18000};
     };
@@ -108,6 +110,12 @@
         int n_mid{};
         long long q_zero_off{};
 
+        std::vector<int> f_static;
+        int n_static_quad{};
+        long long static_root_doubles{};
+        std::vector<int> q_prog_dyn, q_lists_dyn;
+        std::vector<unsigned char> row_keep;
+
         long long nnz_LU{};
         long long nnz_LU_stored{};
         double flops{};
diff --git a/phy-engine_amd/ffi.py b/phy-engine_amd/ffi.py
--- a/phy-engine_amd/ffi.py
+++ b/phy-engine_amd/ffi.py
@@ -28,6 +28,7 @@
     "pe_hip_analyze_tr_adaptive", "pe_hip_get_tr_step_log",
     "pe_hip_analyze_noise", "pe_hip_get_noise", "pe_hip_get_noise_sources", "pe_hip_get_noise_source_density", "pe_hip_get_noise_integrated",
     "pe_hip_set_dc_sweep_rows", "pe_hip_analyze_dc_sweep", "pe_hip_get_dc_sweep", "pe_hip_get_dc_sweep_status",
+    "pe_hip_get_static_fronts", "pe_hip_get_static_skip_stats", "pe_hip_get_static_skip_refinement_stats",
 ]
 DC_SWEEP_PARALLEL, DC_SWEEP_TRACE = 0, 1
 MEAS_MIN, MEAS_MAX, MEAS_AVG, MEAS_RMS, MEAS_INTEG, MEAS_CROSS = 1, 2, 3, 4, 5, 6
@@ -198,6 +199,9 @@
         l.pe_hip_set_options.argtypes = [C.c_void_p, C.POINTER(Options)]
         l.pe_hip_get_info.argtypes = [C.c_void_p, C.POINTER(Info)]
         l.pe_hip_get_front_table.argtypes = [C.c_void_p, C.c_int, C.c_int] + [C.POINTER(C.c_int)] * 9
+        l.pe_hip_get_static_fronts.argtypes = [C.c_void_p, C.c_int, C.c_int, C.POINTER(C.c_int), C.POINTER(C.c_int)]
+        l.pe_hip_get_static_skip_stats.argtypes = [C.c_void_p, C.POINTER(C.c_longlong), C.POINTER(C.c_longlong)]
+        l.pe_hip_get_static_skip_refinement_stats.argtypes = [C.c_void_p, C.POINTER(C.c_longlong), C.POINTER(C.c_longlong)]
         l.pe_hip_set_digital_drives.argtypes = [C.c_void_p, C.c_int, C.POINTER(C.c_int), C.POINTER(C.c_double)]
         l.pe_hip_update_param.argtypes = [C.c_void_p, C.c_int, C.c_int, C.c_int, C.POINTER(C.c_double), C.c_int]
         l.pe_hip_reset.argtypes = [C.c_void_p]
@@ -404,6 +408,20 @@
         self._chk(lib().pe_hip_get_front_table(self._h, int(which), n.value, *[_ip(out[k]) for k in names], C.byref(n)))
         return out
 
+    def static_fronts(self, which=0):
+        n = C.c_int()
+        self._chk(lib().pe_hip_get_static_fronts(self._h, int(which), 0, None, C.byref(n)))
+        out = np.zeros(n.value, dtype=np.int32)
+        self._chk(lib().pe_hip_get_static_fronts(self._h, int(which), n.value, _ip(out), C.byref(n)))
+        return out
+
+    def static_skip_stats(self):
+        a, b = C.c_longlong(), C.c_longlong()
+        self._chk(lib().pe_hip_get_static_skip_stats(self._h, C.byref(a), C.byref(b)))
+        c, d = C.c_longlong(), C.c_longlong()
+        self._chk(lib().pe_hip_get_static_skip_refinement_stats(self._h, C.byref(c), C.byref(d)))
+        return {"skipped_launches": a.value, "full_launches": b.value, "launches_after_refinement": c.value, "skipped_after_refinement": d.value}
+
     def reset(self):
         self._chk(lib().pe_hip_reset(self._h))
 
```

New measurement: 56220 (median of 6 runs). 1.03x the previous value.
